# Sthiber/COSC_4397_Pathtracing_Raytracing_Project

Hardware: AMD Instinct MI355X
Metric: Msamples/s, cornell.txt 1920x1080 depth 8 (+PSNR vs 5000spp ref) (higher is better)
Workload: dtype f32

## Files before the change

cosc_4397_pathtracing_raytracing_project_amd/capi.py:

```python
from __future__ import annotations

import ctypes as C
import math
import os
from typing import Optional, Sequence, Tuple

import numpy as np

_PKG = os.path.dirname(os.path.abspath(__file__))
LIB_PATH = os.environ.get("PT_AMD_LIB") or os.path.join(_PKG, "libpt_amd.so")
PT_MAX_DEPTH = 64
ARITH = {"exact": 0, "fma": 1, "fast": 2}
ARITH_NAMES = {v: k for k, v in ARITH.items()}
FEATURE_PLANES = 3
NOISE_PLANES = 2
NOISE_PIXELS_PER_PARTIAL = 1024
CONVERGENCE_WAVES = 16
CONVERGENCE_CAPACITY = 65536
FLT_MAX = float(np.finfo(np.float32).max)


class PtGeom(C.Structure):
    _fields_ = [("type", C.c_int32), ("materialid", C.c_int32), ("transform", C.c_float * 16),
                ("inverseTransform", C.c_float * 16), ("invTranspose", C.c_float * 16)]


class PtMaterial(C.Structure):
    _fields_ = [("color", C.c_float * 3), ("specular_exponent", C.c_float), ("specular_color", C.c_float * 3),
                ("hasReflective", C.c_float), ("hasRefractive", C.c_float), ("indexOfRefraction", C.c_float),
                ("emittance", C.c_float)]


class PtCamera(C.Structure):
    _fields_ = [("resolution", C.c_int32 * 2), ("position", C.c_float * 3), ("lookAt", C.c_float * 3),
                ("view", C.c_float * 3), ("up", C.c_float * 3), ("right", C.c_float * 3), ("fov", C.c_float * 2),
                ("pixelLength", C.c_float * 2)]


class PtBVHNode(C.Structure):
    _fields_ = [("bmin", C.c_float * 3), ("bmax", C.c_float * 3), ("left", C.c_int32), ("right", C.c_int32),
                ("geomIndex", C.c_int32)]


class PtGridInfo(C.Structure):
    _fields_ = [("res", C.c_int32 * 3), ("origin", C.c_float * 3), ("cell_size", C.c_float * 3), ("pad", C.c_float),
                ("num_cells", C.c_int32), ("num_records", C.c_int32), ("num_leaves", C.c_int32)]


class PtGridRecord(C.Structure):
    _fields_ = [("bmin", C.c_float * 3), ("bmax", C.c_float * 3), ("leaf", C.c_int32), ("neighbours", C.c_int32)]


class PtCameraGridResult(C.Structure):
    _fields_ = [("res", C.c_int32 * 3), ("origin", C.c_float * 3), ("cell_size", C.c_float * 3), ("inv_cell_size", C.c_float * 3), ("pad", C.c_float),
                ("guard", C.c_uint32), ("num_cells", C.c_int64), ("refs", C.c_uint64), ("longest", C.c_uint32), ("status", C.c_int32)]


class PtSceneDesc(C.Structure):
    _fields_ = [("geoms", C.POINTER(PtGeom)), ("num_geoms", C.c_int32), ("materials", C.POINTER(PtMaterial)),
                ("num_materials", C.c_int32), ("camera", PtCamera), ("trace_depth", C.c_int32)]


class PtOptions(C.Structure):
    _fields_ = [("device", C.c_int32), ("pixel_begin", C.c_int32), ("pixel_count", C.c_int32),
                ("iters_per_batch", C.c_int32), ("num_queues", C.c_int32), ("blocks_per_cu", C.c_int32),
                ("time_kernels", C.c_int32), ("legacy_traversal", C.c_int32), ("debug_flags", C.c_int32), ("unfused_primary", C.c_int32), ("unfused_bounces", C.c_int32), ("stripe_pixels", C.c_int32), ("stripe_stride", C.c_int32),
                ("arith", C.c_int32), ("aa_jitter", C.c_int32), ("convergence", C.c_int32),
                ("lds_table_kb", C.c_int32), ("primary_pieces", C.c_int32), ("paths_pieces", C.c_int32), ("paths_min_piece", C.c_int32)]


class PtStats(C.Structure):
    _fields_ = [("samples", C.c_int64), ("live_rays", C.c_int64 * PT_MAX_DEPTH), ("intersect_launches", C.c_int64),
                ("intersect_ms", C.c_double), ("render_ms", C.c_double), ("num_cus", C.c_int32),
                ("grid_blocks", C.c_int32), ("num_queues", C.c_int32), ("iters_per_batch", C.c_int32),
                ("device_bytes", C.c_int64), ("primary_fused", C.c_int32), ("bounces_fused", C.c_int32),
                ("arith", C.c_int32), ("grid_cells", C.c_int32), ("tight_leaves", C.c_int32), ("paths_waves", C.c_int32), ("record_form", C.c_int32),
                ("gather_form", C.c_int32), ("primary_launches", C.c_int64), ("inline_gathers", C.c_int64)]


class PtDenoiseOptions(C.Structure):
    _fields_ = [("levels", C.c_int32), ("sigma_color", C.c_float), ("sigma_normal", C.c_float), ("sigma_position", C.c_float),
                ("keep_albedo", C.c_int32)]


class PtHistoryOptions(C.Structure):
    _fields_ = [("cap", C.c_float), ("min_normal_dot", C.c_float), ("plane_tol", C.c_float), ("keep_view_dependent", C.c_int32)]


class PtHistoryRoundOptions(C.Structure):
    _fields_ = [("min_history", C.c_float), ("max_fraction", C.c_float)]


class PtHistoryProbeOptions(C.Structure):
    _fields_ = [("radius", C.c_int32), ("gain", C.c_float)]


class PtHistoryFeedbackOptions(C.Structure):
    _fields_ = [("level", C.c_int32), ("variance", C.c_int32)]


class PtSetupTimes(C.Structure):
    _fields_ = [("tables_ms", C.c_double), ("upload_ms", C.c_double), ("buffers_ms", C.c_double), ("probe_ms", C.c_double),
                ("set_camera_ms", C.c_double), ("set_camera_calls", C.c_int32)]


class PtSetCameraTimes(C.Structure):
    _fields_ = [("tables_ms", C.c_double), ("rearm_ms", C.c_double), ("total_ms", C.c_double), ("path", C.c_int32), ("fallback", C.c_int32)]


class PtSetGeomsTimes(C.Structure):
    _fields_ = [("build_ms", C.c_double), ("upload_ms", C.c_double), ("rearm_ms", C.c_double), ("total_ms", C.c_double)]


PT_SET_CAMERA_DEVICE_TABLES = 1
PT_DEVICE_TABLES_LIST, PT_DEVICE_TABLES_CELLS = 1, 2
PT_CAMERA_GRID_NONE = 3
TABLE_NODE = np.dtype([("bmin", np.float32, 3), ("bmax", np.float32, 3), ("skip", np.int32), ("geom", np.int32)])
TABLE_NAMES = ("nodes", "nodes_b", "top", "top_b", "grid_start", "grid_items", "grid_items_b", "cull_margin", "geoms")


class PtError(RuntimeError):
    pass


_lib: Optional[C.CDLL] = None
_fp = C.POINTER(C.c_float)
_ip = C.POINTER(C.c_int32)


def lib() -> C.CDLL:
    global _lib
    if _lib is not None:
        return _lib
    if not os.path.exists(LIB_PATH):
        raise PtError(f"{LIB_PATH} not found: run `python -c 'import __graft_entry__ as g; g.build()'` "
                      "(hipcc --offload-arch=gfx950).  There is no CPU fallback.")
    L = C.CDLL(LIB_PATH)
    L.pt_last_error.restype = C.c_char_p
    L.pt_scene_load.argtypes = [C.c_char_p, C.c_int, C.c_int, C.POINTER(C.c_void_p)]
    L.pt_scene_free.argtypes = [C.c_void_p]
    L.pt_scene_free.restype = None
    L.pt_scene_desc.argtypes = [C.c_void_p, C.POINTER(PtSceneDesc)]
    L.pt_scene_iterations.argtypes = [C.c_void_p]
    L.pt_scene_image_name.argtypes = [C.c_void_p]
    L.pt_scene_image_name.restype = C.c_char_p
    L.pt_build_bvh.argtypes = [C.POINTER(PtGeom), C.c_int, C.POINTER(PtBVHNode), C.c_int]
    L.pt_build_grid.argtypes = [C.POINTER(PtGeom), C.c_int, C.c_int, C.POINTER(PtGridInfo), C.POINTER(C.c_uint32), C.POINTER(PtGridRecord)]
    if hasattr(L, "pt_selfcheck_ieee"):
        L.pt_selfcheck_ieee.argtypes = [C.c_int, C.c_int, C.c_uint64, C.c_uint64, C.c_uint32, C.POINTER(C.c_uint64)]
    if hasattr(L, "pt_selfcheck_fast_math"):
        L.pt_selfcheck_fast_math.argtypes = [C.c_int, C.c_int, C.c_uint64, C.c_uint64, C.POINTER(C.c_double)]
    if hasattr(L, "pt_traversal_boxes"):
        L.pt_traversal_boxes.argtypes = [C.POINTER(PtGeom), C.c_int, _fp, _fp]
    if hasattr(L, "pt_center_half_box"):
        L.pt_center_half_box.argtypes = [_fp, _fp, C.c_int, C.c_float, _fp, _fp]
        L.pt_center_half_box.restype = None
    L.pt_build_transform.argtypes = [_fp, _fp, _fp, _fp]
    L.pt_init.argtypes = [C.POINTER(PtSceneDesc), C.POINTER(PtOptions)]
    L.pt_render.argtypes = [C.c_int, C.c_int]
    L.pt_readback.argtypes = [_fp]
    L.pt_readback_device.argtypes = [C.c_void_p]
    L.pt_preview_rgba8.argtypes = [C.c_int, C.POINTER(C.c_uint8)]
    L.pt_preview_rgba8_device.argtypes = [C.c_int, C.c_void_p]
    L.pt_get_stats.argtypes = [C.POINTER(PtStats)]
    L.pt_stage_generate.argtypes = [C.c_int, C.c_int, _fp, _fp]
    L.pt_stage_intersect.argtypes = [C.c_int, _fp, _fp, _fp, _fp, _ip, _fp]
    if hasattr(L, "pt_stage_intersect_grid"):
        L.pt_stage_intersect_grid.argtypes = [C.c_int, _fp, _fp, C.c_int, _fp, _fp, _ip, _fp]
        L.pt_stage_grid_info.argtypes = [C.POINTER(PtGridInfo), C.POINTER(C.c_int32)]
    L.pt_stage_shade.argtypes = [C.c_int, C.c_int, _ip, _ip, _fp, _fp, _ip, _fp, _fp, _fp, _fp, _ip]
    _u8p = C.POINTER(C.c_uint8)
    L.pt_save_u8.argtypes = [C.c_float, _u8p]
    L.pt_stage_save_u8.argtypes = [C.c_int, C.c_int, C.c_float, _fp, _u8p]
    L.pt_ctx_create.argtypes = [C.POINTER(PtSceneDesc), C.POINTER(PtOptions), C.POINTER(C.c_void_p)]
    L.pt_ctx_destroy.argtypes = [C.c_void_p]
    L.pt_ctx_render.argtypes = [C.c_void_p, C.c_int, C.c_int]
    L.pt_ctx_sync.argtypes = [C.c_void_p]
    L.pt_ctx_readback.argtypes = [C.c_void_p, _fp]
    L.pt_ctx_readback_device.argtypes = [C.c_void_p, C.c_void_p]
    L.pt_ctx_save_u8.argtypes = [C.c_void_p, C.c_float, _u8p]
    L.pt_ctx_get_stats.argtypes = [C.c_void_p, C.POINTER(PtStats)]
    L.pt_ctx_reset_stats.argtypes = [C.c_void_p]
    L.pt_ctx_clear.argtypes = [C.c_void_p]
    L.pt_ctx_pixel_count.argtypes = [C.c_void_p]
    L.pt_group_create.argtypes = [C.POINTER(PtSceneDesc), C.POINTER(PtOptions), _ip, C.c_int, C.POINTER(C.c_void_p)]
    if hasattr(L, "pt_group_create_ex"):
        L.pt_group_create_ex.argtypes = [C.POINTER(PtSceneDesc), C.POINTER(PtOptions), _ip, C.c_int, C.c_int, C.POINTER(C.c_void_p)]
        L.pt_group_transport.argtypes = [C.c_void_p]
    L.pt_group_destroy.argtypes = [C.c_void_p]
    L.pt_group_size.argtypes = [C.c_void_p]
    L.pt_group_context.argtypes = [C.c_void_p, C.c_int]
    L.pt_group_context.restype = C.c_void_p
    L.pt_group_render.argtypes = [C.c_void_p, C.c_int, C.c_int]
    L.pt_group_sync.argtypes = [C.c_void_p]
    L.pt_group_gather.argtypes = [C.c_void_p, _fp]
    L.pt_group_gather_u8.argtypes = [C.c_void_p, C.c_float, _u8p]
    L.pt_group_preview_rgba8.argtypes = [C.c_void_p, C.c_int, _u8p]
    L.pt_write_png_rgb8.argtypes = [C.c_char_p, _u8p, C.c_int, C.c_int]
    L.pt_output_basename.argtypes = [C.c_char_p, C.c_int, C.c_char_p, C.c_int]
    L.pt_save_png.argtypes = [C.c_char_p, _fp, C.c_int, C.c_int, C.c_float]
    L.pt_save_hdr.argtypes = [C.c_char_p, _fp, C.c_int, C.c_int, C.c_float]
    L.pt_save_pfm.argtypes = [C.c_char_p, _fp, C.c_int, C.c_int, C.c_float]
    L.pt_load_pfm.argtypes = [C.c_char_p, _fp, C.c_int, _ip, _ip, C.c_float]
    _dp = C.POINTER(C.c_double)
    L.pt_psnr_from_sse.argtypes = [C.c_double, C.c_int64]
    L.pt_psnr_from_sse.restype = C.c_float
    L.pt_set_reference.argtypes = [_fp]
    L.pt_get_convergence.argtypes = [C.c_int, C.c_int, _dp]
    L.pt_iterations_to_clean.argtypes = [C.c_float, _ip]
    L.pt_ctx_set_reference.argtypes = [C.c_void_p, _fp]
    L.pt_ctx_get_convergence.argtypes = [C.c_void_p, C.c_int, C.c_int, _dp]
    L.pt_ctx_iterations_to_clean.argtypes = [C.c_void_p, C.c_float, _ip]
    L.pt_group_set_reference.argtypes = [C.c_void_p, _fp]
    L.pt_group_get_convergence.argtypes = [C.c_void_p, C.c_int, C.c_int, _dp]
    L.pt_group_iterations_to_clean.argtypes = [C.c_void_p, C.c_float, _ip]
    if hasattr(L, "pt_render_features"):
        L.pt_render_features.argtypes = [C.c_int, C.c_int]
        L.pt_readback_features.argtypes = [_fp]
        L.pt_ctx_render_features.argtypes = [C.c_void_p, C.c_int, C.c_int]
        L.pt_ctx_readback_features.argtypes = [C.c_void_p, _fp]
        L.pt_ctx_device_features.argtypes = [C.c_void_p]
        L.pt_ctx_device_features.restype = C.c_void_p
        L.pt_group_render_features.argtypes = [C.c_void_p, C.c_int, C.c_int]
        L.pt_group_gather_features.argtypes = [C.c_void_p, _fp]
    if hasattr(L, "pt_denoise"):
        _dno = C.POINTER(PtDenoiseOptions)
        L.pt_denoise.argtypes = [C.c_float, _dno, _fp]
        L.pt_ctx_denoise.argtypes = [C.c_void_p, C.c_float, _dno, _fp]
        L.pt_ctx_denoise_device.argtypes = [C.c_void_p, C.c_float, _dno, C.POINTER(C.c_void_p)]
        L.pt_group_denoise.argtypes = [C.c_void_p, C.c_float, _dno, _fp]
# ... 1898 lines not shown
```

cosc_4397_pathtracing_raytracing_project_amd/csrc/pt_api.cpp:

```cpp
#include <chrono>
#include <cmath>
#include <cstdarg>
#include <cstdio>
#include <cstring>
#include <string>

#include "pt_adaptive.h"
#include "pt_camera_tables_device.h"
#include "pt_context.h"
#include "pt_lds.h"
#include "pt_scene.h"
#include "pt_sched.h"

namespace {

std::string g_err;
constexpr int kDebugFlags = 16 | 32 | 64 | 256 | 512 | 2048 | ptk::kFormSwitches;
static_assert(sizeof(PtOptions) == 80, "capi.PtOptions mirrors this layout");
static_assert(PT_CONVERGENCE_WAVES == ptk::kConvWaves, "pt_amd.h documents the size of the convergence metric's partial sums");
}
int pt_fail(const char* fmt, ...) {
  char buf[1024];
  va_list ap;
  va_start(ap, fmt);
  vsnprintf(buf, sizeof(buf), fmt, ap);
  va_end(ap);
  g_err = buf;
  return -1;
}

namespace ptc {
static PtContext* g_default = nullptr;
PtContext* default_context() { return g_default; }

int get_events(Ctx& g, EventPair* ev) {
  if (!g.free_events.empty()) {
    *ev = g.free_events.back();
    g.free_events.pop_back();
    return 0;
  }
  HIP_OK(hipEventCreate(&ev->a));
  HIP_OK(hipEventCreate(&ev->b));
  return 0;
}
static int resolve_events(Ctx& g) {
  auto drain = [&](std::vector<EventPair>& pending, double& total_ms) -> int {
    for (auto& e : pending) {
      float ms = 0;
      HIP_OK(hipEventElapsedTime(&ms, e.a, e.b));
      total_ms += ms;
      g.free_events.push_back(e);
    }
    pending.clear();
    return 0;
  };
  g.isect_launches += (int64_t)g.pending_isect.size();
  return drain(g.pending_isect, g.isect_ms) || drain(g.pending_render, g.render_ms) ? -1 : 0;
}

ptk::SceneTables tables(const Ctx& g) {
  ptk::SceneTables t = g.scene;
  if (g.debug_flags & 16) t.cull_margin = INFINITY;
  if (g.debug_flags & 32) t.top_xor = 0;
  t.lds_table_bytes = g.lds_table_bytes;
  t.max_batch_iters = g.K;
  t.trace_depth = g.depth;
  t.scan_nodes_lds = -1;
  t.use_grid = !g.grids.empty() && g.grid_enabled && !(g.debug_flags & 512) ? 1 : 0;
  if (t.use_grid) {
    const Ctx::DeviceGrid& gr = g.grids[g.grid_pick];
    t.lds_table_bytes = -1;
    t.grid_start = gr.d_start + gr.guard;
    t.grid_items = gr.d_items;
    t.grid_items_b = gr.d_items_b;
    for (int a = 0; a < 3; ++a)
      t.grid_res[a] = gr.shape.res[a], t.grid_min[a] = gr.shape.gmin[a], t.grid_cs[a] = gr.shape.cs[a], t.grid_inv_cs[a] = gr.shape.inv_cs[a];
    t.grid_pad = gr.shape.pad;
  }
  return t;
}

static size_t pathbuf_words(int64_t stride) { return (size_t)(2 * stride + (stride * ptd::kPathPlane2Bytes + 15) / 16); }
static int alloc_pathbuf(Ctx& g, ptd::PathBuf* b, int64_t stride) {
  b->stride = stride;
  return dalloc(g, &b->r, pathbuf_words(stride));
}
static int alloc_hitbuf(Ctx& g, ptd::HitBuf* h, int64_t stride) {
  h->stride = stride;
  return dalloc(g, &h->t, stride) || dalloc(g, &h->n, 3 * stride) || dalloc(g, &h->mat, stride) || dalloc(g, &h->p, 3 * stride) ? -1 : 0;
}

static ptd::Queues queues_for(const Ctx& g, int grid) {
  ptd::Queues q = g.qs;
  q.W = grid * ptk::kWavesPerBlock;
  return q;
}

static int primary_share_of(const Ctx& g) { return (g.debug_flags & ptk::kTraceEveryIteration) ? 1 : g.primary_share ? g.primary_share : ptk::kShareMax; }

ptk::BatchInfo tile_batch(const Ctx& g, int iter_first, int K) {
  ptk::BatchInfo b{};
  b.iter_first = iter_first;
  b.K = K;
  b.N = g.N;
  b.pixel_begin = g.pixel_begin;
  b.trace_depth = g.depth;
  b.aa_jitter = g.aa_jitter ? 1 : 0;
  b.stripe = g.stripe;
  b.gap = g.stripe ? g.stripe_stride - g.stripe : 0;
  b.inv_stripe = g.stripe ? 1.0f / (float)g.stripe : 0.0f;
  return b;
}
static ptk::BatchInfo form_batch(const Ctx& g, int iter_first, int K) {
  ptk::BatchInfo b = tile_batch(g, iter_first, K);
  b.slot_shift = g.slot_shift, b.flat = g.fuse_bounces ? 0 : 1, b.primary_share = primary_share_of(g);
  return b;
}

static void gather_waiting(Ctx& g) {
  if (!g.waiting.live) return;
  ptd::RetireBuf ret = g.ret;
  if (g.waiting.plane) ret.rec = g.rec_plane1;
  g.k->collect_stream_planes(g.stream, g.waiting.b, g.qs, ret, g.ret.rec, g.d_image);
  g.waiting.live = false;
}

int run_batch(Ctx& g, int iter_first, int kb, int after) {
  ptk::BatchInfo b = form_batch(g, iter_first, kb);
  b.paths_pieces = g.paths_pieces, b.list = g.list;
  if (b.list) b.stripe = 1, b.gap = 0, b.inv_stripe = 1.0f;
  const ptk::SceneTables sc = tables(g);
  const ptk::BatchForm form = ptk::batch_form(ptk::form_inputs(b, g.debug_flags, ptk::search_form(sc), sc.num_mats, g.ret.seg_cap));
  b.retire_once = form.retire_once, b.split_records = g.record_form = form.records, b.fixed_slots = form.fixed_slots;
  b.primary_pieces = form.shares ? ptk::auto_shared_pieces(kb, g.qs.nq, g.ret.wq0) : ptk::auto_primary_pieces(kb, g.qs.nq, g.ret.wq0);
  if (g.primary_pieces) b.primary_pieces = g.primary_pieces;
  if (form.records == ptk::kFirstBounce) b.primary_pieces = 1;
  const ptk::KernelApi& k = *g.k;
  auto cnt_row = [&](int d) { return g.d_cnt + ptk::cnt_index(g.qs, d, 0); };
  const ptd::Queues pq = queues_for(g, g.grid_primary);
  Ctx::PrimaryKey key;
  std::memset(&key, 0, sizeof(key));
  key.sc = sc, key.cam = g.dcam, key.b = b, key.b.iter_first = key.b.K = 0, key.qs = pq, key.out = g.buf[1], key.ret = g.ret;
  key.kernels = &k, key.grid = g.grid_primary, key.debug_flags = g.debug_flags;
  const bool same_key = form.primary_once && g.primary_valid && std::memcmp(&key, &g.primary_key, sizeof(key)) == 0;
  g.primary_valid = false;
  ptk::ConvInfo cv{g.d_ref, g.d_partial, -1, kb};
  if (g.conv_live) {
    if (g.conv_have_ref) cv.first_k = 0;
    else if (g.conv >= iter_first && g.conv < iter_first + kb) cv.capture_k = g.conv - iter_first, cv.first_k = cv.capture_k + 1, g.conv_have_ref = true;
    g.conv_last = std::max(g.conv_last, iter_first + kb - 1);
  }
  const bool all_depths = g.grid_paths > 0;
  const ptk::GatherPlan plan = ptk::gather_plan({form, cv.capture_k >= 0 || cv.first_k < kb, g.waiting.live, g.waiting.plane, same_key,
                                                 g.rec_plane1 != nullptr && !g.conv, after, g.debug_flags, all_depths});
  ptd::RetireBuf ret = g.ret;
  if (plan.plane) ret.rec = g.rec_plane1;
  if (!plan.gathers_waiting) gather_waiting(g);
  if (!g.fuse_primary) k.generate(g.stream, g.grid_gen, g.dcam, b, queues_for(g, g.grid_gen), g.buf[0], cnt_row(0));
  else if (!same_key) {
    k.primary(g.stream, g.grid_primary, sc, g.dcam, b, pq, cnt_row(0), cnt_row(1), g.buf[1], g.ret);
    g.primary_launches += 1;
    std::memcpy(&g.primary_key, &key, sizeof(key));
  }
  const int d0 = g.fuse_primary ? 1 : 0;
  int src = d0;
  EventPair ev{};
  auto timed_from = [&]() -> int {
    if (!g.time_kernels) return 0;
    if (get_events(g, &ev)) return -1;
    HIP_OK(hipEventRecord(ev.a, g.stream));
    return 0;
  };
  auto timed_to = [&]() -> int {
    if (!g.time_kernels) return 0;
    HIP_OK(hipEventRecord(ev.b, g.stream));
    g.pending_isect.push_back(ev);
    return 0;
  };
  if (all_depths) {
    if (timed_from()) return -1;
    if (plan.gathers_waiting) {
      const ptk::PrevGather prev{g.waiting.plane ? g.rec_plane1 : g.ret.rec, g.ret.rec, g.d_image, g.waiting.b.K, 0};
      k.paths_gather(g.stream, g.grid_paths, sc, b, queues_for(g, g.grid_paths), g.d_cnt, g.buf[1], ret, prev);
      g.waiting.live = false;
      g.inline_gathers += 1;
    } else k.paths(g.stream, g.grid_paths, sc, b, queues_for(g, g.grid_paths), g.d_cnt, g.buf[1], ret);
    if (timed_to()) return -1;
  }
  for (int d = d0; d < g.depth && !all_depths; ++d) {
    const int32_t* cin = cnt_row(d);
    int32_t* cout = cnt_row(d + 1);
    if (timed_from()) return -1;
    k.intersect(g.stream, g.grid_isect, sc, queues_for(g, g.grid_isect), cin, g.buf[src], g.hits, g.legacy, d == 0);
    if (timed_to()) return -1;
    k.shade(g.stream, g.grid_shade, sc, b, d, queues_for(g, g.grid_shade), cin, cout, g.buf[src], g.hits, g.buf[src ^ 1], g.ret);
    src ^= 1;
  }
  g.gather_form = plan.reported;
  if (plan.closing == ptk::kCloseStream) k.collect_stream(g.stream, b, g.qs, g.ret, g.d_image, g.d_cnt, g.depth, g.d_stats);
  else k.count_stats(g.stream, g.qs, g.d_cnt, g.depth, g.d_stats);
  if (plan.closing == ptk::kCloseStatsStreamPlanes) k.collect_stream_planes(g.stream, b, g.qs, ret, g.ret.rec, g.d_image);
  if (plan.closing == ptk::kCloseStatsConv) k.collect_conv(g.stream, b, g.qs, g.ret, g.d_image, cv, g.d_sse);
  if (plan.closing == ptk::kCloseStatsTile) k.collect(g.stream, b, g.qs, g.ret, g.d_image);
  if (plan.defers) g.waiting.live = true, g.waiting.b = b, g.waiting.plane = plan.plane;
  HIP_OK(hipGetLastError());
  g.primary_valid = form.primary_once;
  g.samples += (int64_t)kb * g.N;
  if (g.pending_isect.size() > 16384) {
    HIP_OK(hipStreamSynchronize(g.stream));
    if (resolve_events(g)) return -1;
  }
  return 0;
}

void plan_launch(Ctx& g) {
  if (!g.borrowed) g.lds_table_bytes = g.k->lds_table_limit(tables(g), g.lds_table_forced);
  const ptk::SceneTables t = tables(g);
  g.grid_gen = g.num_cus * std::min(g.cap_bpc, g.k->resident_blocks_per_cu(ptk::kGenerate, t));
  g.grid_isect = g.num_cus * std::min(g.cap_bpc, g.k->resident_blocks_per_cu(g.legacy ? ptk::kIntersectLegacy : ptk::kIntersect, t));
  g.grid_shade = g.num_cus * std::min(g.cap_bpc, g.k->resident_blocks_per_cu(ptk::kShade, t));
  g.grid_primary = g.num_cus * std::min(g.cap_bpc, g.k->resident_blocks_per_cu(ptk::primary_shares(form_batch(g, 0, g.K)) ? ptk::kPrimaryShared : ptk::kPrimary, t));
  g.ret.wq0 = ptk::wave_slot(0, g.qs.Q, g.grid_primary * ptk::kWavesPerBlock).wq;
  g.grid_paths = (g.fuse_bounces && g.depth > 1) ? g.num_cus * std::min(g.cap_bpc, g.k->resident_blocks_per_cu(ptk::kPaths, t)) : 0;
  g.qs.paths_W = g.grid_paths * ptk::kWavesPerBlock;
  g.primary_valid = false;
}

static void free_grid(Ctx& g, const Ctx::DeviceGrid& d) {
  for (void* p : {(void*)d.d_start, (void*)d.d_items, d.d_items_b != d.d_items ? (void*)d.d_items_b : nullptr}) {
    if (!p) continue;
    (void)hipFree(p);
    g.allocs.erase(std::remove(g.allocs.begin(), g.allocs.end(), p), g.allocs.end());
  }
  g.device_bytes -= (int64_t)d.bytes;
}
static int choose_traversal(Ctx& g) {
  auto drop_unused_grids = [&](size_t keep) {
    for (size_t i = 0; i < g.grids.size(); ++i)
      if (i != keep) free_grid(g, g.grids[i]);
    g.grids = {g.grids[keep]};
    g.grid_pick = 0;
  };
  if (g.grids.empty()) return 0;
  if (!g.fuse_bounces || (g.debug_flags & (256 | 512))) {
    drop_unused_grids(0);
    return 0;
  }
// ... 104 lines not shown
  auto pieces = [](int v, int automatic) { return v ? std::clamp(v, 1, 0x7fff) : automatic; };
  g.lds_table_forced = opt.lds_table_kb ? std::clamp(opt.lds_table_kb, 0, ptk::kLdsTableBytes / 1024) * 1024 : -1;
  g.primary_pieces = pieces(opt.primary_pieces < 0 ? opt.primary_pieces : opt.primary_pieces & 0xffff, 0);
  g.primary_share = opt.primary_pieces < 0 ? 0 : std::min(opt.primary_pieces >> 16 & 0x7f, ptk::kShareMax);
  g.paths_pieces = ptk::pack_paths_pieces(pieces(opt.paths_pieces, 2), pieces(opt.paths_min_piece, 64));
  g.fuse_primary = !g.legacy && !opt.unfused_primary;
  g.fuse_bounces = g.fuse_primary && !opt.unfused_bounces;
  g.cap_bpc = opt.blocks_per_cu > 0 ? std::min(opt.blocks_per_cu, 8) : 8;
}

int batch_iters_for(int iters_per_batch, int N, int* slot_shift) {
  int K = iters_per_batch;
  if (K <= 0) {
    const int64_t target = 48ll << 20;
    K = (int)std::max<int64_t>(1, std::min<int64_t>(256, (target + N - 1) / N));
  }
  int shift = 1;
  while ((1ll << shift) < N) ++shift;
  if (shift > 30) return pt_fail("pt_init: tiles of more than 2^30 pixels are not supported");
  while (K > 1 && K > (1 << (31 - shift))) --K;
  if (slot_shift) *slot_shift = shift;
  return K;
}

int plan_batches(Ctx& g, const PtOptions& opt) {
  const int W = g.cam.resolution[0], H = g.cam.resolution[1];
  g.opt_iters_per_batch = opt.iters_per_batch, g.opt_num_queues = opt.num_queues;
  g.pixel_begin = opt.pixel_begin;
  g.N = opt.pixel_count > 0 ? opt.pixel_count : W * H - opt.pixel_begin;
  g.stripe = opt.stripe_pixels;
  g.stripe_stride = opt.stripe_stride;
  if (g.stripe < 0 || (g.stripe > 0 && g.stripe_stride < g.stripe)) return pt_fail("pt_init: bad stripe %d / stride %d", g.stripe, g.stripe_stride);
  {
    int64_t last = (int64_t)g.pixel_begin + g.N - 1;
    if (g.stripe > 0) last = (int64_t)g.pixel_begin + (g.N - 1) + (int64_t)((g.N - 1) / g.stripe) * (g.stripe_stride - g.stripe);
    if (g.pixel_begin < 0 || g.N <= 0 || last >= (int64_t)W * H)
      return pt_fail("pt_init: tile [%d, +%d, stripe %d/%d) outside %dx%d", opt.pixel_begin, opt.pixel_count, g.stripe, g.stripe_stride, W, H);
    if (g.stripe > 0 && g.N / g.stripe >= 32768) return pt_fail("pt_init: more than 32767 stripes");
    if (H >= 32768) return pt_fail("pt_init: image height %d not supported (>= 32768)", H);
  }
  const int K = batch_iters_for(opt.iters_per_batch, g.N, &g.slot_shift);
  if (K < 0) return -1;

  int Q = opt.num_queues > 0 ? opt.num_queues : 256;
  const int cu_waves = g.num_cus * ptk::kWavesPerBlock;
  if (Q > cu_waves) Q = cu_waves;
  while (cu_waves % Q) --Q;
  if (opt.num_queues <= 0)
    while (ptk::chunks_per_queue(g.N, Q) > 128 && 2 * Q <= cu_waves && cu_waves % (2 * Q) == 0) Q *= 2;
  const ptk::QueuePlan plan = ptk::queue_plan(g.N, Q, K);
  const int grid = g.num_cus * 8;
  g.K = K;
  g.grid = grid;
  g.qs.Q = Q;
  g.qs.W = grid * ptk::kWavesPerBlock;
  g.qs.cnt_stride = 16;
  g.qs.nq = plan.nq;
  g.qs.inv_nq = 1.0f / (float)plan.nq;
  g.qs.cap = plan.cap;
  g.stride = (int64_t)Q * g.qs.cap;
  g.ret.seg_cap = plan.seg_cap;
  g.ret.kmax = K;
  return 0;
}

template <typename T>
static const T* upload(Ctx& g, const std::vector<T>& v) {
  T* p = nullptr;
  if (dalloc(g, &p, v.size())) return nullptr;
  const hipError_t e = hipMemcpy(p, v.data(), v.size() * sizeof(T), hipMemcpyHostToDevice);
  return e == hipSuccess ? p : (pt_fail("hipMemcpy(%zu bytes) failed: %s", v.size() * sizeof(T), hipGetErrorString(e)), nullptr);
}
static int upload_grid(Ctx& g, const pt::Grid& gr) {
  Ctx::DeviceGrid d{gr.shape, gr.guard, nullptr, nullptr, nullptr, 0, gr.start};
  const int64_t before = g.device_bytes;
  if (!(d.d_start = upload(g, gr.start)) || !(d.d_items = upload(g, gr.items))) return -1;
  if (!(d.d_items_b = gr.items_b.empty() ? d.d_items : upload(g, gr.items_b))) return -1;
  d.bytes = (size_t)(g.device_bytes - before);
  d.items = gr.items.size();
  g.grids.push_back(d);
  return 0;
}
static int upload_tables(Ctx& g, const pt::HostTables& t) {
  ptk::SceneTables& s = g.scene;
  s.num_nodes = (int)t.nodes.size(), s.num_geoms = (int)t.geoms.size(), s.num_mats = (int)t.mats.size(), s.num_top = (int)t.top.size();
  std::memcpy(s.root_min, t.root_min, 12);
  std::memcpy(s.root_max, t.root_max, 12);
  s.cull_margin = t.cull_margin;
  s.top_xor = t.top_xor;
  s.has_triangles = t.has_triangles ? 1 : 0;
  g.tight_leaves = t.tight_leaves;
  if (!(s.nodes = upload(g, t.nodes)) || !(s.geoms = upload(g, t.geoms)) || !(s.mats = upload(g, t.mats)) || !(s.top = upload(g, t.top))) return -1;
  s.nodes_b = s.nodes, s.top_b = s.top;
  if (!t.nodes_b.empty() && (!(s.nodes_b = upload(g, t.nodes_b)) || !(s.top_b = upload(g, t.top_b)))) return -1;
  for (const pt::Grid& gr : t.grids)
    if (upload_grid(g, gr)) return -1;
  return 0;
}

static __global__ void k_poison_records(ptd::Word4* rec, unsigned long long per_queue, unsigned long long total, int Q) {
  const float nan = __builtin_nanf("");
  for (unsigned long long i = (unsigned long long)blockIdx.x * blockDim.x + threadIdx.x; i < total; i += (unsigned long long)gridDim.x * blockDim.x)
    rec[i] = ptd::Word4{nan, nan, nan, __int_as_float(ptk::chunk_pixel((int)(i / per_queue), 0, Q))};
}

static int poison_records(Ctx& g) {
  const size_t regions = (size_t)g.qs.Q * g.ret.kmax, per_queue = (size_t)g.ret.kmax * g.ret.seg_cap;
  for (ptd::Word4* plane : {g.ret.rec, g.rec_plane1})
    if (plane)
      hipLaunchKernelGGL(k_poison_records, dim3((unsigned)std::min<size_t>((regions * g.ret.seg_cap + 255) / 256, 65536)), dim3(256), 0, g.stream, plane,
                         (unsigned long long)per_queue, (unsigned long long)(regions * g.ret.seg_cap), g.qs.Q);
  HIP_OK(hipGetLastError());
  return 0;
}
static size_t sub_words_max(const Ctx& g) { return ptk::sub_stride(g.num_cus * 8 * ptk::kWavesPerBlock, g.qs.Q); }

static int rearm_batch_buffers(Ctx& g) {
  g.primary_valid = false;
  for (const ptd::PathBuf& pb : g.buf) HIP_OK(hipMemsetAsync(pb.r, 0xff, pathbuf_words(pb.stride) * sizeof(ptd::Word4), g.stream));
  const size_t regions = (size_t)g.qs.Q * g.ret.kmax;
  HIP_OK(hipMemsetAsync(g.ret.cnt, 0, regions * sizeof(*g.ret.cnt), g.stream));
  HIP_OK(hipMemsetAsync(g.ret.sub, 0, regions * sub_words_max(g) * sizeof(*g.ret.sub), g.stream));
  if (g.qs.deal) HIP_OK(hipMemsetAsync(g.qs.deal, 0, (size_t)ptk::deal_map(g.qs).words() * sizeof(int32_t), g.stream));
  return poison_records(g);
}

int alloc_batch_buffers(Ctx& g) {
  const int Q = g.qs.Q;
  if (alloc_pathbuf(g, &g.buf[0], g.stride) || alloc_pathbuf(g, &g.buf[1], g.stride)) return -1;
  for (const ptd::PathBuf& pb : g.buf) HIP_OK(hipMemset(pb.r, 0xff, pathbuf_words(pb.stride) * sizeof(ptd::Word4)));
  if (!g.fuse_bounces && alloc_hitbuf(g, &g.hits, g.stride)) return -1;
  {
    const size_t regions = (size_t)Q * g.ret.kmax;
    const size_t wq_max = sub_words_max(g);
    if (dalloc(g, &g.ret.rec, regions * g.ret.seg_cap)) return -1;
    g.rec_plane1 = nullptr;
    if (g.fuse_primary && g.fuse_bounces && g.depth > 1 && !g.aa_jitter && !g.borrowed && !(g.debug_flags & ptk::kNoSecondPlane)) {
      void* p = nullptr;
      const size_t bytes = regions * g.ret.seg_cap * sizeof(ptd::Word4);
      if (hipMalloc(&p, bytes) == hipSuccess) {
        g.allocs.push_back(p);
        g.device_bytes += (int64_t)bytes;
        g.rec_plane1 = static_cast<ptd::Word4*>(p);
      } else (void)hipGetLastError();
    }
    if (ensure(g, g.ret.cnt, regions * sizeof(*g.ret.cnt), Zero::blocking) || ensure(g, g.ret.sub, regions * wq_max * sizeof(*g.ret.sub), Zero::blocking)) return -1;
    if (poison_records(g)) return -1;
  }
  const size_t image_bytes = 3 * (size_t)g.N * sizeof(float);
  const size_t cnt_words = ptk::cnt_index(g.qs, g.depth + 1, 0);
  if (ensure(g, g.d_image, image_bytes, Zero::blocking) || ensure(g, g.d_cnt, cnt_words * sizeof(int32_t), Zero::blocking) ||
      ensure(g, g.d_stats, PT_MAX_DEPTH * sizeof(*g.d_stats), Zero::blocking))
    return -1;
  if (!(g.debug_flags & 64) && ensure(g, g.qs.deal, (size_t)ptk::deal_map(g.qs).words() * sizeof(int32_t), Zero::blocking)) return -1;
  if (g.conv) {
    const size_t partials = (size_t)g.K * Q * ptk::kConvWaves;
    if (ensure(g, g.d_ref, image_bytes, Zero::blocking) || ensure(g, g.d_partial, partials * sizeof(double), Zero::blocking)) return -1;
    if (dalloc(g, &g.d_sse, (size_t)PT_CONVERGENCE_CAPACITY)) return -1;
    HIP_OK(hipMemset(g.d_sse, 0xff, (size_t)PT_CONVERGENCE_CAPACITY * sizeof(double)));
  }
  HIP_OK(hipDeviceSynchronize());
  return 0;
}

static int setup(Ctx& g, const PtSceneDesc* sc, const PtOptions& opt) {
  if (open_device(g, opt)) return -1;
  take_scene_and_options(g, sc, opt);
  if (plan_batches(g, opt)) return -1;
  if ((size_t)sc->num_materials * sizeof(ptd::Mat) > 60 * 1024) return pt_fail("pt_init: %zu materials exceed the LDS table", (size_t)sc->num_materials);
  using clock = std::chrono::steady_clock;
  auto ms_since = [](clock::time_point t0) { return std::chrono::duration<double, std::milli>(clock::now() - t0).count(); };
  clock::time_point t0 = clock::now();
  const pt::HostTables host = pt::build_scene_tables(*sc, g.debug_flags, g.k->boxes_center_half != 0, pt::GridRequest{}, &g.camera_base);
  g.setup_times.tables_ms = ms_since(t0), t0 = clock::now();
  if (upload_tables(g, host)) return -1;
  g.setup_times.upload_ms = ms_since(t0), t0 = clock::now();
  plan_launch(g);
  if (alloc_batch_buffers(g)) return -1;
  g.setup_times.buffers_ms = ms_since(t0), t0 = clock::now();
  if (choose_traversal(g)) return -1;
  g.setup_times.probe_ms = ms_since(t0);
  g.grid_request.kind = pt::GridRequest::kNone;
  if (tables(g).use_grid) {
    g.grid_request.kind = pt::GridRequest::kFixed;
    std::memcpy(g.grid_request.res, g.grids[g.grid_pick].shape.res, sizeof(g.grid_request.res));
  }
  g.time_kernels = opt.time_kernels != 0;
  g.conv_live = g.conv != 0;
  return 0;
}

int need(const PtContext* c, const char* who) { return c ? 0 : pt_fail("%s: pt_init has not been called", who); }

int admit(const PtContext& g, const char* who, unsigned req) {
  if ((req & kNotFailed) && g.failed) return pt_fail("%s: an earlier batch of this context failed (%s); free it and create a new one", who, g_err.c_str());
  if ((req & kUniform) && g.adaptive)
    return pt_fail("%s: the renderer is in the adaptive state (pt_adaptive_round): one sample count no longer describes the image; read it with pt_resolve, or "
                   "return to the uniform state with pt_clear", who);
  if ((req & kNoExtras) && g.hist_extra)
    return pt_fail("%s: the history round left extra samples in some pixels (pt_history_round): one sample count no longer describes the image; read it with "
                   "pt_history_resolve, or return to the uniform state with pt_clear", who);
  const int W = g.cam.resolution[0];
  if ((req & kWholeRows) && (g.stripe || g.pixel_begin % W || g.N % W))
    return pt_fail("%s: the tile must consist of whole contiguous image rows (begin %d, count %d, stripe %d, width %d)", who, g.pixel_begin, g.N, g.stripe, W);
  if ((req & kFoldedAll) && g.rendered != g.noise_iters)
    return pt_fail("%s: %lld iteration(s) rendered since the last fold; fold first (pt_noise_fold)", who, (long long)(g.rendered - g.noise_iters));
  if (req & kOnDevice) HIP_OK(hipSetDevice(g.device));
  return 0;
}

}
using namespace ptc;

extern "C" {

const char* pt_last_error(void) { return g_err.c_str(); }

int pt_selfcheck_ieee(int arith, int kind, uint64_t first, uint64_t count, uint32_t seed, uint64_t* mismatches) {
  const ptk::KernelApi* k = ptk::api_for(arith);
  if (!k || kind < 0 || kind > 4 || !mismatches) return pt_fail("pt_selfcheck_ieee: bad argument");
  unsigned long long* d = nullptr;
  HIP_OK(hipMalloc(&d, sizeof(*d)));
  hipError_t e = hipMemset(d, 0, sizeof(*d));
  if (e == hipSuccess) {
    k->ieee_check(nullptr, kind, first, count, seed, d);
    e = hipGetLastError();
  }
  unsigned long long h = 0;
  if (e == hipSuccess) e = hipMemcpy(&h, d, sizeof(h), hipMemcpyDeviceToHost);
  (void)hipFree(d);
  if (e != hipSuccess) return pt_fail("pt_selfcheck_ieee: %s", hipGetErrorString(e));
  *mismatches = h;
  return 0;
}

int pt_selfcheck_fast_math(int arith, int kind, uint64_t first, uint64_t count, double* max_err) {
  const ptk::KernelApi* k = ptk::api_for(arith);
  if (!k || kind < 0 || kind > 8 || !max_err) return pt_fail("pt_selfcheck_fast_math: bad argument");
  unsigned long long* d = nullptr;
  HIP_OK(hipMalloc(&d, sizeof(*d)));
  hipError_t e = hipMemset(d, 0, sizeof(*d));
  if (e == hipSuccess) {
    k->fast_math_check(nullptr, kind, first, count, d);
    e = hipGetLastError();
  }
  unsigned long long h = 0;
  if (e == hipSuccess) e = hipMemcpy(&h, d, sizeof(h), hipMemcpyDeviceToHost);
  (void)hipFree(d);
  if (e != hipSuccess) return pt_fail("pt_selfcheck_fast_math: %s", hipGetErrorString(e));
  std::memcpy(max_err, &h, sizeof(h));
  return 0;
}

struct PtScene {
  pt::Scene scene;
  explicit PtScene(const std::string& f) : scene(f) {}
};

int pt_scene_load(const char* path, int res_w, int res_h, PtScene** out) {
  if (!path || !out) return pt_fail("pt_scene_load: null argument");
  try {
    PtScene* s = new PtScene(path);
    if (res_w > 0 && res_h > 0) s->scene.overrideResolution(res_w, res_h);
    s->scene.applyInitialCameraState();
    *out = s;
    return 0;
  } catch (const std::exception& e) {
    return pt_fail("pt_scene_load: %s", e.what());
  }
}
void pt_scene_free(PtScene* s) { delete s; }
int pt_scene_desc(const PtScene* s, PtSceneDesc* out) {
  if (!s || !out) return pt_fail("pt_scene_desc: null argument");
  *out = s->scene.desc();
  return 0;
}
int pt_scene_orbit(PtScene* s, float dphi, float dtheta, float dzoom) {
  if (!s) return pt_fail("pt_scene_orbit: null scene");
  s->scene.orbit(dphi, dtheta, dzoom);
  return 0;
}
int pt_scene_camera(const PtScene* s, PtCamera* out) {
  if (!s || !out) return pt_fail("pt_scene_camera: null argument");
  *out = s->scene.state.camera;
  return 0;
}
int pt_scene_orbit_state(const PtScene* s, float* phi, float* theta, float* zoom) {
  if (!s) return pt_fail("pt_scene_orbit_state: null scene");
  if (phi) *phi = s->scene.phi;
  if (theta) *theta = s->scene.theta;
  if (zoom) *zoom = s->scene.zoom;
  return 0;
}
static int scene_geom(const PtScene* s, int geom, const void* trs, const char* who) {
  if (!s || !trs) return pt_fail("%s: null argument", who);
  if (geom < 0 || (size_t)geom >= s->scene.geoms.size()) return pt_fail("%s: geom %d is outside the scene's %zu geoms", who, geom, s->scene.geoms.size());
  if (s->scene.geom_trs[(size_t)geom].mesh) return pt_fail("%s: geom %d is a triangle of a mesh object: its vertices are world-space, it has no TRS of its own", who, geom);
  return 0;
}
int pt_scene_geom_trs(const PtScene* s, int geom, float trs[9]) {
  if (scene_geom(s, geom, trs, "pt_scene_geom_trs")) return -1;
  std::memcpy(trs, s->scene.geom_trs[(size_t)geom].trs, 9 * sizeof(float));
  return 0;
}
int pt_scene_set_geom_trs(PtScene* s, int geom, const float trs[9]) {
  if (scene_geom(s, geom, trs, "pt_scene_set_geom_trs")) return -1;
  for (int k = 0; k < 9; ++k)
// ... 59 lines not shown
  if (!sc) return pt_fail("pt_init: null scene");
  if (sc->num_geoms <= 0 || !sc->geoms) return pt_fail("pt_init: scene has no geometry");
  if (sc->num_materials <= 0 || !sc->materials) return pt_fail("pt_init: scene has no materials");
  if (sc->trace_depth <= 0 || sc->trace_depth > PT_MAX_DEPTH) return pt_fail("pt_init: trace_depth %d out of range", sc->trace_depth);
  const int W = sc->camera.resolution[0], H = sc->camera.resolution[1];
  if (W <= 0 || H <= 0 || (int64_t)W * H > (1ll << 30)) return pt_fail("pt_init: bad resolution %dx%d", W, H);
  for (int i = 0; i < sc->num_geoms; ++i) {
    if (sc->geoms[i].materialid < 0 || sc->geoms[i].materialid >= sc->num_materials)
      return pt_fail("pt_init: geom %d references material %d of %d", i, sc->geoms[i].materialid, sc->num_materials);
    if (sc->geoms[i].type < PT_GEOM_SPHERE || sc->geoms[i].type > PT_GEOM_TRIANGLE)
      return pt_fail("pt_init: geom %d has unknown type %d", i, sc->geoms[i].type);
  }
  PtOptions opt{};
  if (opt_in) opt = *opt_in;
  PtContext* c = new PtContext();
  if (setup(*c, sc, opt)) {
    destroy(c);
    return -1;
  }
  *out = c;
  return 0;
}

int pt_ctx_destroy(PtContext* c) {
  if (c == g_default) g_default = nullptr;
  destroy(c);
  return 0;
}

int pt_ctx_render(PtContext* c, int iter_first, int iter_count) {
  if (need(c, "pt_render")) return -1;
  if (iter_count <= 0) return 0;
  Ctx& g = *c;
  if (admit(g, "pt_render", kNotFailed | kUniform)) return -1;
  if (g.conv_live) {
    if (iter_first < 1 || (int64_t)iter_first + iter_count - 1 > PT_CONVERGENCE_CAPACITY)
      return pt_fail("pt_render: iterations %d .. %lld outside 1 .. %d (PT_CONVERGENCE_CAPACITY) with the convergence metric on", iter_first,
                  (long long)iter_first + iter_count - 1, PT_CONVERGENCE_CAPACITY);
    if (g.conv < 0 && !g.conv_have_ref) return pt_fail("pt_render: PtOptions.convergence is -1 but no reference frame has been supplied (pt_set_reference)");
  }
  HIP_OK(hipSetDevice(g.device));
  EventPair ev{};
  if (get_events(g, &ev)) return -1;
  HIP_OK(hipEventRecord(ev.a, g.stream));
  const int end = iter_first + iter_count;
  for (int it = iter_first; it < end; it += g.K)
    if (run_batch(g, it, std::min(g.K, end - it), it + g.K < end ? (end - it - 1) / g.K : 0)) {
      g.failed = true;
      g.free_events.push_back(ev);
      return -1;
    }
  HIP_OK(hipEventRecord(ev.b, g.stream));
  g.pending_render.push_back(ev);
  g.rendered += iter_count;
  g.fb_pending = false;
  return 0;
}

int pt_ctx_sync(PtContext* c) {
  if (need(c, "pt_sync")) return -1;
  HIP_OK(hipSetDevice(c->device));
  HIP_OK(hipStreamSynchronize(c->stream));
  return resolve_events(*c);
}

int pt_ctx_readback(PtContext* c, float* out) {
  if (need(c, "pt_readback")) return -1;
  return copy_out(c, "pt_readback", out, 3, [&](const float** d) { return *d = c->d_image, 0; });
}

int pt_ctx_readback_device(PtContext* c, void* out) {
  if (need(c, "pt_readback_device")) return -1;
  return copy_out(c, "pt_readback_device", static_cast<float*>(out), 3, [&](const float** d) { return *d = c->d_image, 0; }, hipMemcpyDeviceToDevice);
}

const float* pt_ctx_device_image(PtContext* c) { return c ? c->d_image : nullptr; }
void* pt_ctx_stream(PtContext* c) { return c ? (void*)c->stream : nullptr; }
int pt_ctx_pixel_count(const PtContext* c) { return c ? c->N : 0; }
int pt_ctx_device(const PtContext* c) { return c ? c->device : -1; }

int pt_ctx_save_u8_device(PtContext* c, float samples, const uint8_t** rgb8_dev) {
  if (need(c, "pt_save_u8")) return -1;
  Ctx& g = *c;
  const int W = g.cam.resolution[0];
  if (!(samples > 0.0f)) return pt_fail("pt_save_u8: samples must be positive");
  if (admit(g, "pt_save_u8", kUniform | kNoExtras)) return -1;
  if (g.pixel_begin % W || g.N % W || (g.stripe && g.stripe != W))
    return pt_fail("pt_save_u8: the tile must consist of whole image rows (begin %d, count %d, stripe %d, width %d)", g.pixel_begin, g.N, g.stripe, W);
  HIP_OK(hipSetDevice(g.device));
  if (ensure(g, g.d_rgb8, 3 * (size_t)g.N)) return -1;
  g.k->save_u8(g.stream, g.N, W, samples, g.d_image, g.d_rgb8);
  HIP_OK(hipGetLastError());
  if (rgb8_dev) *rgb8_dev = g.d_rgb8;
  return 0;
}
int pt_ctx_save_u8(PtContext* c, float samples, uint8_t* rgb8_host) {
  return copy_out(c, "pt_save_u8", rgb8_host, 3, [&](const uint8_t** d) { return pt_ctx_save_u8_device(c, samples, d); });
}

int pt_ctx_preview_rgba8_device(PtContext* c, int iterations, void* rgba_dev) {
  if (need(c, "pt_preview_rgba8_device")) return -1;
  if (!rgba_dev || iterations <= 0) return pt_fail("pt_preview_rgba8_device: bad argument");
  if (admit(*c, "pt_preview_rgba8_device", kUniform | kNoExtras | kOnDevice)) return -1;
  c->k->preview(c->stream, c->N, iterations, c->d_image, reinterpret_cast<uchar4*>(rgba_dev));
  HIP_OK(hipStreamSynchronize(c->stream));
  return 0;
}

int pt_ctx_preview_rgba8(PtContext* c, int iterations, uint8_t* rgba_host) {
  if (need(c, "pt_preview_rgba8")) return -1;
  if (!rgba_host || iterations <= 0) return pt_fail("pt_preview_rgba8: bad argument");
  if (admit(*c, "pt_preview_rgba8", kUniform | kNoExtras | kOnDevice)) return -1;
  uchar4* d = nullptr;
  HIP_OK(hipMalloc((void**)&d, (size_t)c->N * 4));
  c->k->preview(c->stream, c->N, iterations, c->d_image, d);
  hipError_t e = hipMemcpyAsync(rgba_host, d, (size_t)c->N * 4, hipMemcpyDeviceToHost, c->stream);
  if (e == hipSuccess) e = hipStreamSynchronize(c->stream);
  (void)hipFree(d);
  if (e != hipSuccess) return pt_fail("pt_preview_rgba8: %s", hipGetErrorString(e));
  return 0;
}

int pt_ctx_get_stats(PtContext* c, PtStats* out) {
  if (need(c, "pt_get_stats")) return -1;
  if (!out) return pt_fail("pt_get_stats: null");
  if (pt_ctx_sync(c)) return -1;
  Ctx& g = *c;
  std::memset(out, 0, sizeof(*out));
  unsigned long long st[PT_MAX_DEPTH];
  HIP_OK(hipMemcpy(st, g.d_stats, sizeof(st), hipMemcpyDeviceToHost));
  for (int d = 0; d < PT_MAX_DEPTH; ++d) out->live_rays[d] = (int64_t)st[d];
  out->samples = g.samples;
  out->intersect_launches = g.isect_launches;
  out->intersect_ms = g.isect_ms;
  out->render_ms = g.render_ms;
  out->num_cus = g.num_cus;
  out->grid_blocks = g.grid_paths > 0 ? g.grid_paths : g.grid_isect;
  out->num_queues = g.qs.Q;
  out->iters_per_batch = g.K;
  out->device_bytes = g.device_bytes;
  out->primary_fused = g.fuse_primary ? 1 : 0;
  out->bounces_fused = g.fuse_bounces ? 1 : 0;
  out->arith = g.arith;
  if (tables(g).use_grid && g.fuse_bounces) {
    const int* res = g.grids[g.grid_pick].shape.res;
    out->grid_cells = res[0] * res[1] * res[2];
  }
  out->tight_leaves = g.tight_leaves;
  out->record_form = g.record_form;
  out->gather_form = g.gather_form;
  out->inline_gathers = g.inline_gathers;
  out->primary_launches = g.primary_launches;
  out->paths_waves = 0;
  if (g.qs.deal && g.grid_paths > 0) {
    const ptk::DealMap dm = ptk::deal_map(g.qs);
    std::vector<int32_t> first((size_t)dm.made_for() + 1);
    HIP_OK(hipMemcpy(first.data(), g.qs.deal + dm.first(0), first.size() * sizeof(int32_t), hipMemcpyDeviceToHost));
    if (first[dm.made_for()] == g.qs.paths_W) {
      int lo = first[1] - first[0], hi = lo;
      for (int q = 1; q < g.qs.Q; ++q) lo = std::min(lo, first[q + 1] - first[q]), hi = std::max(hi, first[q + 1] - first[q]);
      out->paths_waves = std::min(lo, 0xffff) << 16 | std::min(hi, 0xffff);
    }
  }
  return 0;
}

int pt_ctx_reset_stats(PtContext* c) {
  if (need(c, "pt_reset_stats")) return -1;
  if (pt_ctx_sync(c)) return -1;
  Ctx& g = *c;
  HIP_OK(hipMemsetAsync(g.d_stats, 0, PT_MAX_DEPTH * sizeof(unsigned long long), g.stream));
  HIP_OK(hipStreamSynchronize(g.stream));
  g.samples = 0;
  g.isect_ms = g.render_ms = 0;
  g.isect_launches = 0;
  return 0;
}

int pt_ctx_clear(PtContext* c) {
  if (need(c, "pt_clear")) return -1;
  if (pt_ctx_sync(c)) return -1;
  HIP_OK(hipMemsetAsync(c->d_image, 0, 3 * (size_t)c->N * sizeof(float), c->stream));
  if (c->d_feat) HIP_OK(hipMemsetAsync(c->d_feat, 0, (size_t)PT_FEATURE_PLANES * c->N * sizeof(float4), c->stream));
  if (c->d_noise) HIP_OK(hipMemsetAsync(c->d_noise, 0, pt_noise_state_bytes((size_t)c->N), c->stream));
  c->noise_groups = 0;
  c->noise_iters = c->rendered = 0;
  if (c->d_acnt) HIP_OK(hipMemsetAsync(c->d_acnt, 0, (size_t)c->N * sizeof(ptad::Cnt), c->stream));
  c->adaptive = false;
  c->adaptive_rounds = 0;
  c->adaptive_last = 0;
  c->hist_current = c->feat_fresh = false;
  c->hist_var_current = 0;
  c->fb_current = c->fb_pending = false;
  if (c->d_hist_extra) HIP_OK(hipMemsetAsync(c->d_hist_extra, 0, (size_t)c->N * sizeof(float), c->stream));
  c->hist_extra = false;
  c->hist_noise = c->hist_ne = false;
  c->probe_checked = c->probe_applied = false;
  if (c->conv) {
    HIP_OK(hipMemsetAsync(c->d_sse, 0xff, (size_t)PT_CONVERGENCE_CAPACITY * sizeof(double), c->stream));
    c->conv_last = 0;
    if (c->conv > 0) c->conv_have_ref = false;
  }
  return pt_ctx_reset_stats(c);
}

}
int pt_ctx_camera_refusal(const PtContext* c, const PtCamera* cam, const char* who) {
  if (need(c, who) || admit(*c, who, kNotFailed)) return -1;
  if (!cam) return pt_fail("%s: null camera", who);
  if (cam->resolution[0] != c->cam.resolution[0] || cam->resolution[1] != c->cam.resolution[1])
    return pt_fail("%s: resolution %dx%d differs from the renderer's %dx%d; a new resolution needs pt_init", who, cam->resolution[0], cam->resolution[1],
                   c->cam.resolution[0], c->cam.resolution[1]);
  const struct {
    const char* name;
    const float* v;
    int n;
  } fields[] = {{"position", cam->position, 3}, {"view", cam->view, 3}, {"up", cam->up, 3}, {"right", cam->right, 3}, {"fov", cam->fov, 2}, {"pixelLength", cam->pixelLength, 2}};
  for (const auto& f : fields)
    for (int i = 0; i < f.n; ++i)
      if (!std::isfinite(f.v[i])) return pt_fail("%s: camera %s[%d] is not finite", who, f.name, i);
  return 0;
}
int pt_ctx_camera_refusal_ex(const PtContext* c, const PtCamera* cam, uint32_t flags, const char* who) {
  if (need(c, who) || admit(*c, who, kNotFailed)) return -1;
  if (!cam) return pt_fail("%s: null camera", who);
  if (flags & ~(uint32_t)PT_SET_CAMERA_DEVICE_TABLES) return pt_fail("%s: undefined flag bit(s) 0x%x (defined: PT_SET_CAMERA_DEVICE_TABLES = 0x%x)", who, flags & ~(uint32_t)PT_SET_CAMERA_DEVICE_TABLES, PT_SET_CAMERA_DEVICE_TABLES);
  return pt_ctx_camera_refusal(c, cam, who);
}
int pt_ctx_geoms_refusal(const PtContext* c, const PtGeom* geoms, int num_geoms, const char* who) {
  if (need(c, who) || admit(*c, who, kNotFailed)) return -1;
  if (!geoms) return pt_fail("%s: null geoms", who);
  const std::vector<PtGeom>& have = c->camera_base.geoms;
  if (num_geoms != (int)have.size())
    return pt_fail("%s: %d geoms, but the renderer was created with %d; adding or removing objects needs pt_init", who, num_geoms, (int)have.size());
  for (int i = 0; i < num_geoms; ++i)
    if (geoms[i].type != have[(size_t)i].type || geoms[i].materialid != have[(size_t)i].materialid)
      return pt_fail("%s: geom %d has type %d and material %d, the renderer's has type %d and material %d; only the transforms may change", who, i, geoms[i].type,
                     geoms[i].materialid, have[(size_t)i].type, have[(size_t)i].materialid);
  for (int i = 0; i < num_geoms; ++i)
    for (const float* m : {geoms[i].transform, geoms[i].inverseTransform, geoms[i].invTranspose})
      for (int k = 0; k < 16; ++k)
        if (!std::isfinite(m[k])) return pt_fail("%s: geom %d has a matrix element that is not finite", who, i);
  return 0;
}
namespace {
template <typename T>
void release(Ctx& g, const T* dev, size_t count) {
  if (!dev) return;
  void* p = const_cast<T*>(dev);
  (void)hipFree(p);
  g.allocs.erase(std::remove(g.allocs.begin(), g.allocs.end(), p), g.allocs.end());
  g.device_bytes -= (int64_t)std::max<size_t>(count * sizeof(T), 16);
}
template <typename T>
int reupload(const T* dev, const std::vector<T>& v) {
  HIP_OK(hipMemcpy(const_cast<T*>(dev), v.data(), v.size() * sizeof(T), hipMemcpyHostToDevice));
  return 0;
}
int move_grid(Ctx& g, const pt::Grid* gr) {
  if (!g.grids.empty()) {
    Ctx::DeviceGrid& d = g.grids[g.grid_pick];
    if (gr && gr->start.size() == d.start.size() && gr->items.size() == d.items && gr->items_b.empty() == (d.d_items_b == d.d_items)) {
      if (reupload(d.d_start, gr->start) || reupload(d.d_items, gr->items)) return -1;
      if (!gr->items_b.empty() && reupload(d.d_items_b, gr->items_b)) return -1;
      d.shape = gr->shape, d.guard = gr->guard, d.start = gr->start, d.start_stale = false;
      return 0;
    }
    free_grid(g, d);
    g.grids.clear();
    g.grid_pick = 0;
  }
  return gr ? upload_grid(g, *gr) : 0;
}
int move_tables(Ctx& g) {
  pt::HostTables t;
  std::memcpy(t.root_min, g.scene.root_min, 12);
  std::memcpy(t.root_max, g.scene.root_max, 12);
  const bool center_half = g.k->boxes_center_half != 0;
  pt::camera_tables(t, g.camera_base, g.cam.position, g.debug_flags, center_half, g.grid_request);
  ptk::SceneTables& s = g.scene;
  if (reupload(s.nodes, t.nodes) || reupload(s.top, t.top)) return -1;
  if (center_half && (reupload(s.nodes_b, t.nodes_b) || reupload(s.top_b, t.top_b))) return -1;
  s.cull_margin = t.cull_margin;
  g.tight_leaves = t.tight_leaves;
  return move_grid(g, t.grids.empty() ? nullptr : &t.grids[0]);
}


int ensure_device_base(Ctx& g) {
  Ctx::DeviceBase& b = g.device_base;
  if (b.ready) return 0;
  const pt::CameraBase& cb = g.camera_base;
  std::vector<ptct::DeviceGeom> geoms(cb.geoms.size());
  for (size_t i = 0; i < geoms.size(); ++i) {
    geoms[i] = ptct::DeviceGeom{};
    std::memcpy(geoms[i].inv, cb.geoms[i].inverseTransform, sizeof(geoms[i].inv));
    geoms[i].type = cb.geoms[i].type;
  }
  if (!(b.nodes = upload(g, cb.nodes)) || !(b.top = upload(g, cb.top)) || !(b.geoms = upload(g, geoms))) return -1;
  if (b.rec) return b.ready = true, 0;
  if (dalloc(g, &b.rec, 1)) return -1;
  if (g.grid_request.kind == pt::GridRequest::kFixed) {
    int64_t ncell = 1, leaves = 0;
    for (int a = 0; a < 3; ++a) ncell *= std::min(512, std::max(1, g.grid_request.res[a]));
    for (const ptd::Node& n : cb.nodes) leaves += n.geom >= 0 ? 1 : 0;
    if (ncell <= ptct::kDeviceMaxCells) {
// ... 400 lines not shown
```

cosc_4397_pathtracing_raytracing_project_amd/csrc/pt_device.h:

```cpp
#pragma once
#include <stdint.h>

namespace ptd {

struct Node {
  float bmin[3];
  float bmax[3];
  int32_t skip;
  int32_t geom;
};
static_assert(sizeof(Node) == 32, "Node must be 32 B");

constexpr int kMaxTop = 32;
struct TopEntry {
  float bmin[3];
  float bmax[3];
  int32_t idx;
  int32_t link;
};
static_assert(sizeof(TopEntry) == 32, "TopEntry must be 32 B");

struct Geom {
  float inv[12];
  float xf[12];
  float invT[12];
  int32_t type;
  int32_t material;
  int32_t pad[2];
  float box_normal[7][4];
};
static_assert(sizeof(Geom) == 272, "Geom must be 272 B");

struct Mat {
  float color[3];
  float spec[3];
  float reflective;
  float refractive;
  float emittance;
  float pad[3];
};
static_assert(sizeof(Mat) == 48, "Mat must be 48 B");

struct Camera {
  int32_t res_x, res_y;
  float pos[3], view[3], up[3], right[3];
  float pl_x, pl_y;
};

struct alignas(16) Word4 {
  float x, y, z, w;
};
constexpr int kPathPlane2Bytes = 8;
struct PathBuf {
  Word4* r;
  int64_t stride;
};
struct HitBuf {
  float* t;
  float* n;
  int32_t* mat;
  float* p;
  int64_t stride;
};

struct RetireBuf {
  Word4* rec;
  unsigned long long* sub;
  unsigned long long* cnt;
  int32_t seg_cap;
  int32_t kmax;
  int32_t wq0;
  int32_t pad;
};

struct Queues {
  int32_t Q;
  int32_t cap;
  int32_t W;
  int32_t cnt_stride;
  int32_t nq;
  float inv_nq;
  int32_t* deal;
  int32_t paths_W;
  int32_t pad;
};

}
```

cosc_4397_pathtracing_raytracing_project_amd/csrc/pt_kernels.hip:

```cpp
#include "pt_kernels.h"

#include <float.h>

#include <type_traits>

#include "pt_lds.h"
#include "pt_sched.h"
#include "pt_portable_math.h"

#ifndef PT_ARITH
#define PT_ARITH 0
#endif
#if PT_ARITH == 0
#define PT_NS arith_exact
#define PT_API_FN api_exact
#elif PT_ARITH == 1
#define PT_NS arith_fma
#define PT_API_FN api_fma
#elif PT_ARITH == 2
#define PT_NS arith_fast
#define PT_API_FN api_fast
#else
#error "PT_ARITH must be 0, 1 or 2"
#endif
// ... 1186 lines not shown
      "global_load_lds_dwordx4 %[o16], %[b1]\n\t"
      "s_add_u32 m0, m0, 0x400\n\t"
      "s_nop 0\n\t"
      "global_load_lds_dword %[o8], %[b2]\n\t"
      "s_add_u32 m0, m0, 0xfc\n\t"
      "s_nop 0\n\t"
      "global_load_lds_dword %[o8], %[b2] offset:4\n\t"
      "s_mov_b32 m0, %[keep]"
      : [keep] "=&s"(keep)
      : [base] "s"(lds_base), [b0] "s"(b0), [b1] "s"(b1), [b2] "s"(b2), [o16] "v"(off16), [o8] "v"(off8)
      : "memory", "scc");
}
PT_DEV void fetch_split_to_lds(const void* b0, const void* b1, int i, int i0, uint32_t lds_base) {
  uint32_t keep;
  const uint32_t off = (uint32_t)i << 4, off0 = (uint32_t)i0 << 4;
  asm volatile(
      "s_mov_b32 %[keep], m0\n\t"
      "s_mov_b32 m0, %[base]\n\t"
      "s_nop 0\n\t"
      "global_load_lds_dwordx4 %[o], %[b0]\n\t"
      "s_add_u32 m0, m0, 0x400\n\t"
      "s_nop 0\n\t"
      "global_load_lds_dwordx4 %[o0], %[b1]\n\t"
      "s_mov_b32 m0, %[keep]"
      : [keep] "=&s"(keep)
      : [base] "s"(lds_base), [b0] "s"(b0), [b1] "s"(b1), [o] "v"(off), [o0] "v"(off0)
      : "memory", "scc");
}
PT_DEV void read_record_slot(uint32_t s16, uint32_t s4, v4f& w0, v4f& w1, float& cz, int& nslot, int& nrs) {
  asm volatile(
      "s_waitcnt vmcnt(0)\n\t"
      "ds_read_b128 %0, %5\n\t"
      "ds_read_b128 %1, %5 offset:1024\n\t"
      "ds_read_b32 %2, %6\n\t"
      "ds_read_b32 %3, %6 offset:256\n\t"
      "ds_read_b32 %4, %6 offset:512\n\t"
      "s_waitcnt lgkmcnt(0)"
      : "=&v"(w0), "=&v"(w1), "=&v"(cz), "=&v"(nslot), "=&v"(nrs)
      : "v"(s16), "v"(s4)
      : "memory");
}
struct Lanes {
  unsigned long long* best;
  float* rec;
  uint16_t* ent;
  int head, count;
  int appended, processed;
};
PT_DEV Lanes lanes_init(char* base) {
  Lanes c;
  c.best = reinterpret_cast<unsigned long long*>(base + LanesMap::best);
  c.rec = reinterpret_cast<float*>(base + LanesMap::rec);
  c.ent = reinterpret_cast<uint16_t*>(base + LanesMap::ent);
  c.head = c.count = c.appended = c.processed = 0;
  return c;
}
PT_DEV void paths_chunk(Lanes& c, int n, int lane, f3 o, f3 d, const uint32_t* tword, const ptd::Geom* __restrict__ geoms) {
  const bool valid = lane < n;
  const uint32_t entry = c.ent[(c.head + lane) & (kRing - 1)];
  const int src = (int)(entry & 63u);
  const uint32_t tw = tword[valid ? entry >> 6 : 0u];
  const uint32_t leaf = tw & 255u;
  const f3 ro = mk(bperm(src, o.x), bperm(src, o.y), bperm(src, o.z));
  const f3 rd = mk(bperm(src, d.x), bperm(src, d.y), bperm(src, d.z));
  const ptd::Geom* G = geoms + (valid ? (int)(tw >> 8) : 0);
  f3 pt = mk(0.f, 0.f, 0.f), nrm = mk(0.f, 0.f, 0.f);
  const float t = geom_test<-1, false>(G, ro, rd, pt, nrm, mk(0.f, 0.f, 0.f));
  const uint32_t tb = __float_as_uint(t);
  if (valid && t > 0.f && tb < 0x7f7fffffu) {
    const unsigned long long key = ((unsigned long long)tb << 32) | leaf;
    unsigned long long* slot = &c.best[src];
    atomicMin(slot, key);
    if (*slot == key) {
      float* r = c.rec + src;
      r[0 * 64] = nrm.x, r[1 * 64] = nrm.y, r[2 * 64] = nrm.z;
      r[3 * 64] = pt.x, r[4 * 64] = pt.y, r[5 * 64] = pt.z;
    }
  }
  c.head = (c.head + n) & (kRing - 1);
  c.count -= n;
  c.processed += n;
}
typedef __attribute__((address_space(4))) const v4f cfloat4;
template <typename TOP>
PT_DEV void paths_search(Lanes& c, TOP* top, const uint32_t* tword, int ntop, const ptd::Geom* __restrict__ geoms, f3 o, f3 d,
                         bool fresh, int lane, int& mark) {
  const RayInv ri = ray_inv(d, o);
  if (fresh) {
    c.best[lane] = kNoHit;
    mark = c.processed;
  }
  uint32_t mask = 0;
  for (int e0 = 0; e0 < ntop; e0 += 8) {
#pragma unroll
    for (int u = 0; u < 8; ++u) {
      const int e = e0 + u;
      if (e < ntop) {
        const auto A = top[2 * e], B = top[2 * e + 1];
        mask = push_bit(mask, slab(o, ri, A.x, A.y, A.z, A.w, B.x, B.y));
      }
    }
  }
  mask = fresh ? mask : 0u;
  while (true) {
    const unsigned long long m = ballot(mask != 0u);
    if (!m) break;
    const int rank = rank_in(m);
    if (mask != 0u) {
      const int te = ntop - 1 - __builtin_ctz(mask);
      mask &= mask - 1u;
      c.ent[(c.head + c.count + rank) & (kRing - 1)] = (uint16_t)((te << 6) | lane);
      if (mask == 0u) mark = c.appended + rank + 1;
    }
    const int cnt = __popcll(m);
    c.count += cnt;
    c.appended += cnt;
    if (c.count >= 64) paths_chunk(c, 64, lane, o, d, tword, geoms);
  }
}
constexpr int kPathsScanWaves = 5, kPathsGridWaves = 5;
constexpr int kVisitLap = 32, kVisitsPerRefill = 31;
static_assert(kVisitLap + kVisitsPerRefill + 1 <= kVisitRing, "the visit ring laps a path in flight");
static_assert((kVisitRing & (kVisitRing - 1)) == 0, "visit numbers wrap with a mask");
constexpr int kInlineGroup = 8;
template <int GROUP>
PT_DEV void stream_gather_slot(int N, int K, const QueueShare& sh, const ptd::RetireBuf& ret, const ptd::Word4* plane, const ptd::Word4* front,
                               float* __restrict__ image, int q, int s);
template <typename... PREV>
struct PathsPrev {};
template <typename P>
struct PathsPrev<P> {
  P p;
};
template <typename... PREV>
struct PathsArgs {
  SceneTables sc;
  BatchInfo b;
  ptd::Queues qs;
  int32_t* cnt;
  ptd::PathBuf in;
  ptd::RetireBuf ret;
  PathsPrev<PREV...> prev;
};
template <typename A>
PT_DEV const A& cold_args() {
  auto p = __builtin_amdgcn_kernarg_segment_ptr();
  asm volatile("" : "+s"(p));
  return *(const A*)p;
}
PT_DEV int cold(int v) {
  asm volatile("" : "+s"(v));
  return v;
}
template <Search MODE, int SPLIT = 0, typename... PREV>
__global__ __launch_bounds__(kBlock, MODE == 0 ? kPathsWaves : MODE == 1 ? kPathsScanWaves : kPathsGridWaves) void k_paths(SceneTables sc, BatchInfo b, ptd::Queues qs, int32_t* __restrict__ cnt ,
                                                               ptd::PathBuf in, ptd::RetireBuf ret, PREV... prev) {
  extern __shared__ float4 lds_raw[];
  char* lds = reinterpret_cast<char*>(lds_raw);
  const PathsLds L = paths_lds<MODE, kFast>(sc);
  stage16(lds + L.top, sc.top_b, MODE == 2 ? 0 : top_bytes(sc));
  stage16(lds + L.mats, sc.mats, mat_bytes(sc));
  const float4* top = reinterpret_cast<const float4*>(lds + L.top);
  const ptd::Mat* mats = reinterpret_cast<const ptd::Mat*>(lds + L.mats);
  const ptd::Node* nodes = sc.nodes_b;
  const ptd::Geom* geoms = sc.geoms;
  if (MODE == 0) {
    stage16(lds + L.geoms, sc.geoms, geom_bytes(sc));
    geoms = reinterpret_cast<const ptd::Geom*>(lds + L.geoms);
  }
  const char* lnodes = nullptr;
  if (MODE == 1 && sc.scan_nodes_lds > 0) {
    stage16(lds + L.nodes, sc.nodes_b, node_bytes(sc));
    lnodes = lds + L.nodes;
  }
  using WM = PathsWaveMap<MODE, kFast>;
  constexpr bool FIXED = SPLIT == kFixedSlots, FIRST = SPLIT == kFirstBounce || FIXED;
  constexpr bool GATHER = sizeof...(PREV) > 0;
  static_assert(!GATHER || FIXED, "only a batch with fixed record slots gathers its predecessor");
  constexpr bool COLD = MODE == kLdsTables;
  using Args = PathsArgs<PREV...>;
  auto c_b = [&]() -> const BatchInfo& {
    if constexpr (COLD) return cold_args<Args>().b;
    else return b;
  };
  auto c_qs = [&]() -> const ptd::Queues& {
    if constexpr (COLD) return cold_args<Args>().qs;
    else return qs;
  };
  const int he = iter_hash_entries(sc);
  uint32_t* tword = reinterpret_cast<uint32_t*>(lds + L.tword);
  int* lmat = reinterpret_cast<int*>(lds + L.lmat);
  uint32_t* ihash = reinterpret_cast<uint32_t*>(lds + L.ihash);
  for (int d = 1; d < b.trace_depth; ++d) iter_hash_fill(ihash + (d - 1) * he, sc, b, d);
  for (int e = threadIdx.x; MODE == 0 && e < sc.num_top; e += blockDim.x) {
    const int leaf = sc.top[e].idx, gi = sc.nodes[leaf].geom;
    tword[e] = (uint32_t)leaf | ((uint32_t)gi << 8);
    lmat[leaf & 63] = sc.geoms[gi].material;
  }
  __syncthreads();
  const int wib = threadIdx.x >> 6;
  char* wbase = lds + L.waves + wib * L.wave_bytes;
  Lanes cy = lanes_init(wbase);
  GridRings gr = grid_rings_init<false>(wbase);
  Carry<false, 1>& cb = gr.cy;
  CellRing& cr = gr.cr;
  cb.lnodes = (const __attribute__((address_space(3))) v4f*)(lnodes ? lnodes : lds), cb.lds_nodes = lnodes != nullptr;
  constexpr bool SLOTS = MODE == 0;
  char* slots = wbase + WM::slots;
  int* died = reinterpret_cast<int*>(wbase + WM::died);
  [[maybe_unused]] int* fillc = reinterpret_cast<int*>(wbase + WM::fillc);
  const int ntop = sc.num_top;
  const int wave = __builtin_amdgcn_readfirstlane(blockIdx.x * kWavesPerBlock + wib);
  const int lane = lane_id();
  died[lane] = 0;
  const uint64_t t_begin = __builtin_amdgcn_s_memrealtime();
  const DealMap dm = deal_map(qs);
  const WaveSlot even = wave_slot(wave, qs.Q, qs.W);
  int q = even.q, r = even.r, wq = even.wq;
  if (qs.deal != nullptr && qs.deal[dm.made_for()] == qs.W) {
    int at_or_before = 0;
    for (int e0 = 0; e0 < qs.Q; e0 += 64) at_or_before += (int)__popcll(ballot(e0 + lane < qs.Q && qs.deal[dm.first(e0 + lane)] <= wave));
    q = at_or_before - 1;
    const int first = qs.deal[dm.first(q)];
    r = wave - first, wq = qs.deal[dm.first(q + 1)] - first;
  }
  const Retire rt = retire_of(ret, q);
  const int64_t qbase = (int64_t)q * qs.cap;
  const int wq0 = rt.wq0, ne = b.K * wq0;
  const QueueShare qshare = queue_share(b, qs, q);
  const int my_nq = qshare.my_nq, quo = my_nq / wq0, rem = my_nq % wq0;
  auto count_of = [&](int e) { return e < ne ? (int)(uint32_t)rt.sub[e] : 0; };
  int total = 0, csum = 0;
  const bool chunk_sums = ne <= 64 * 64;
  for (int e0 = 0; e0 < ne; e0 += 256) {
    int n4[4];
#pragma unroll
    for (int j = 0; j < 4; ++j) n4[j] = count_of(e0 + 64 * j + lane);
#pragma unroll
    for (int j = 0; j < 4; ++j) {
      int sum;
      (void)wave_prefix6(n4[j], sum);
      total += sum;
      if (lane == (e0 >> 6) + j) csum = sum;
    }
  }
  if (r == 0 && lane == 0) cnt[cnt_index(qs, 1, q)] = total;
  if constexpr (SPLIT == kFirstBounce || SPLIT == kFixedSlots)
    if (r == 0 && lane == 0) cnt[cnt_index(qs, 0, q)] = b.K * qshare.my_pixels;
  const PiecePlan pieces0 = piece_plan(total, wq, b.paths_pieces, qs.deal != nullptr, chunk_sums);
  auto piece_plan_here = [&]() {
    if constexpr (COLD) return piece_plan(cold(total), wq, c_b().paths_pieces, c_qs().deal != nullptr, cold(ne) <= 64 * 64);
    else return pieces0;
  };
  [[maybe_unused]] int clist0 = 0;
  int ce = ne, cstart = total, ccnt = 0, clist = 0;
  int cord = 0;
  [[maybe_unused]] int cur_k = 0;
  [[maybe_unused]] uint32_t cur_h = 0u, next_h = 0u;
  [[maybe_unused]] int crec0 = 0;
  [[maybe_unused]] const int fbits = fixed_bits(rt.seg_cap);
  int win0 = -64;
  unsigned long long wsub = 0ull;
  auto window_to = [&](int e) {
    if (e < win0 || e >= win0 + 64) {
      win0 = e;
      wsub = (e + lane < ne) ? rt.sub[e + lane] : 0ull;
    }
  };
  auto sub_word = [&](int e) -> unsigned long long {
    const uint32_t lo32 = (uint32_t)__builtin_amdgcn_readlane((int)(uint32_t)wsub, e - win0);
    const uint32_t hi32 = (uint32_t)__builtin_amdgcn_readlane((int)(uint32_t)(wsub >> 32), e - win0);
    return ((unsigned long long)hi32 << 32) | lo32;
  };
  window_to(0);
  auto cursor_bases = [&](int first_rank) {
    const int ec = min(ce, ne - 1), ck = ec / wq0, crho = ec - ck * wq0;
    clist = ck * rt.seg_cap + sub_offset(quo, rem, crho) * 64;
    if constexpr (SPLIT != 0) clist0 = invariant_slot(clist, ck, rt.seg_cap);
    if constexpr (FIRST) cur_k = ck, cur_h = iter_hash(b.iter_first + ck, 0);
    window_to(ec);
    const int crec = clist + (int)(uint32_t)(sub_word(ec) >> 32);
    if constexpr (FIXED) crec0 = invariant_slot(crec, ck, rt.seg_cap);
    else if (lane == 0) fillc[cord & (kVisitRing - 1)] = crec + (first_rank - cstart);
  };
  auto seek = [&](int at_rank) {
    int cum = 0, e_begin = 0;
    if (COLD ? cold(ne) <= 64 * 64 : chunk_sums) {
      int all;
      const int cbefore = wave_prefix6(csum, all);
      const unsigned long long here = ballot(csum > 0 && cbefore <= at_rank && at_rank < cbefore + csum);
      if (here) {
        const int l = __builtin_ctzll(here);
        e_begin = l * 64, cum = __builtin_amdgcn_readlane(cbefore, l);
      }
    }
    for (int e0 = e_begin; e0 < ne; e0 += 64) {
      const int n = count_of(e0 + lane);
      int sum;
      const int before = wave_prefix6(n, sum);
      const unsigned long long here = ballot(n > 0 && cum + before <= at_rank && at_rank < cum + before + n);
      if (here) {
        const int l = __builtin_ctzll(here);
        ce = e0 + l, cstart = cum + __builtin_amdgcn_readlane(before, l), ccnt = __builtin_amdgcn_readlane(n, l);
        break;
      }
      cum += sum;
    }
    ++cord;
    cursor_bases(at_rank);
  };
  auto assign = [&](bool want, int rank, int& at, [[maybe_unused]] int& at0, int& rs) -> bool {
    bool pending = want;
    const int cord0 = cord;
    while (true) {
      const bool in = pending && rank < cstart + ccnt;
      if (in) at = clist + (rank - cstart), rs = cord;
      if constexpr (SPLIT != 0)
        if (in) at0 = clist0 + (rank - cstart);
      if constexpr (FIRST)
        if (in) rs = (int)(FIXED ? pack_fixed(cur_k, crec0 + (rank - cstart), fbits) : pack_visit(cur_k, cord)), next_h = cur_h;
      pending = pending && !in;
      if (!ballot(pending) || ce >= ne || (!FIXED && cord - cord0 >= kVisitsPerRefill)) break;
      cstart += ccnt;
      ccnt = 0;
      int nxt = ce + 1;
      while (nxt < ne) {
        window_to(nxt);
        const unsigned long long holds = ballot((uint32_t)wsub != 0u) & (~0ull << (nxt - win0));
        if (holds) {
          nxt = win0 + (int)__builtin_ctzll(holds);
          ccnt = (int)(uint32_t)sub_word(nxt);
          break;
        }
        nxt = win0 + 64;
      }
      ce = min(nxt, ne);
      ++cord;
      cursor_bases(cstart);
    }
    return want && !pending;
  };
  const uint32_t s_base = (uint32_t)__builtin_amdgcn_readfirstlane((int)lds_offset(slots));
  const uint32_t s16 = s_base + (uint32_t)lane * 16u, s4 = s_base + (uint32_t)kSlotTail + (uint32_t)lane * 4u;
  const ptd::Word4 *in0 = uniform_ptr(in.r + qbase), *in1 = uniform_ptr(in.r + in.stride + qbase);
  const float* in2 = uniform_ptr(reinterpret_cast<const float*>(in.r + 2 * in.stride) + 2 * qbase);
  PathRec nx;
  nx.o = nx.d = nx.c = mk(0.f, 0.f, 0.f), nx.tag = PathTag{0, 0u, 0};
  int nx_rs = 0;
  int* slot_rs = reinterpret_cast<int*>(slots + kSlotVisit) + lane;
  auto fetch = [&](int at, [[maybe_unused]] int at0, int rs) {
    if constexpr (SLOTS && SPLIT == kSplitRecords) fetch_split_to_lds(in0, in1, at, at0, s_base), *slot_rs = rs;
    else if constexpr (SLOTS) fetch_record_to_lds(in0, in1, in2, FIRST ? at0 : at, s_base), *slot_rs = rs;
    else if constexpr (SPLIT == kSplitRecords) {
      const ptd::Word4 w0 = in.r[qbase + at], w1 = in.r[in.stride + qbase + at0];
      nx.o = mk(w0.x, w0.y, w0.z), nx.d = mk(w0.w, w1.x, w1.y), nx.c = mk(w1.z, w1.w, 0.f), nx_rs = rs;
    } else nx = path_load(in, qbase + at), nx_rs = rs;
  };
  const int pix0 = b.stripe == 0 && b.pixel_begin >= 0 ? b.pixel_begin : -1;
  auto refill_pixel_map = [&]() {
    PixelMap pm{0, 0, 0, 0.f, nullptr};
    if constexpr (COLD)
      if (pix0 < 0) pm = pixel_map(c_b());
    return pm;
  };
  auto pixel_of = [&](const PixelMap& pm, int pl) {
    if constexpr (COLD) {
      if (pix0 >= 0) return pix0 + pl;
      return global_pixel(pm, pl);
    } else return global_pixel(b, pl);
  };
  [[maybe_unused]] uintptr_t top_b_scalar = (uintptr_t)sc.top_b;
  if constexpr (COLD && kFast) asm volatile("" : "+s"(top_b_scalar));
  f3 o = mk(0.f, 0.f, 0.f), d = o, c = o;
  int slot = 0, depth = 1, mark = 0, rslot = 0;
  uint32_t phash = 0u;
  bool valid = false, fresh = false, owes = false;
  bool has_next = false;
  int streamed = 0, p_hi = 0;
  [[maybe_unused]] int gj = r;
  [[maybe_unused]] uint32_t gather_time = 0u;
  [[maybe_unused]] auto gather_step = [&]() {
    if constexpr (GATHER) {
      const Args& ka = cold_args<Args>();
      const PrevGather& pg = ka.prev.p;
      const int gq = cold(q);
      const uint64_t t0 = __builtin_amdgcn_s_memrealtime();
      stream_gather_slot<kInlineGroup>(ka.b.N, pg.K, queue_share(ka.b, ka.qs, gq), ka.ret, pg.rec, pg.plane0, pg.image, gq, gj * 64 + lane);
      gj += wq;
      gather_time += (uint32_t)(__builtin_amdgcn_s_memrealtime() - t0);
    }
  };
  while (!FIRST) {
    if (streamed >= p_hi && p_hi >= 0) {
      const PiecePlan pieces = piece_plan_here();
      int nextp = -1;
      if (cord == 0) nextp = r;
      else if (pieces.needs_counter()) {
        int v = 0;
        if (lane == 0) v = atomicAdd(&c_qs().deal[deal_map(c_qs()).piece_counter(q)], 1);
        nextp = wq + __builtin_amdgcn_readfirstlane(v);
      }
      const PieceRange pr = pieces.piece_range(nextp);
      if (pr.some) {
        streamed = pr.start, p_hi = pr.end;
        seek(streamed);
      } else {
        p_hi = -1;
      }
    }
    const bool take = !valid && has_next;
    if (ballot(take || owes || (!valid && !has_next && streamed < p_hi))) {
      const PixelMap pm = refill_pixel_map();
      v4f w0, w1;
      float cz;
      int nslot, nrs;
      if constexpr (SLOTS && SPLIT == kSplitRecords) {
        asm volatile(
            "s_waitcnt vmcnt(0)\n\t"
            "ds_read_b128 %0, %3\n\t"
            "ds_read_b128 %1, %3 offset:1024\n\t"
            "ds_read_b32 %2, %4 offset:512\n\t"
            "s_waitcnt lgkmcnt(0)"
            : "=&v"(w0), "=&v"(w1), "=&v"(nrs)
            : "v"(s16), "v"(s4)
            : "memory");
        cz = 0.f, nslot = 0;
      } else if constexpr (SLOTS) {
        read_record_slot(s16, s4, w0, w1, cz, nslot, nrs);
      } else {
        w0 = v4f{nx.o.x, nx.o.y, nx.o.z, nx.d.x}, w1 = v4f{nx.d.y, nx.d.z, nx.c.x, nx.c.y}, cz = nx.c.z, nslot = nx.tag.slot, nrs = nx_rs;
      }
      if (owes) {
        rt.rec[rslot] = ptd::Word4{c.x, c.y, c.z, __int_as_float(slot & ((1 << b.slot_shift) - 1))};
        owes = false;
      }
      if constexpr (SPLIT == kSplitRecords) {
        if (take) {
          const uint32_t word = __float_as_uint(w0.w);
          const ptd::Mat* m = mats + __float_as_int(w1.w);
          nslot = kind_sample_id(word);
          o = mk(w1.x, w1.y, w1.z), d = mk(w0.x, w0.y, w0.z);
          c = mul(mk(1.0f, 1.0f, 1.0f), kind_specular(word) ? mk(m->spec[0], m->spec[1], m->spec[2]) : mk(m->color[0], m->color[1], m->color[2]));
        }
      } else if (take) o = mk(w0.x, w0.y, w0.z), d = mk(w0.w, w1.x, w1.y), c = mk(w1.z, w1.w, cz);
      if (take) {
        slot = nslot, rslot = nrs;
        phash = utilhash((uint32_t)pixel_of(pm, nslot & ((1 << b.slot_shift) - 1)));
        depth = 1;
        valid = fresh = true;
        has_next = false;
      }
      const bool lapping = ballot(valid && cord - rslot >= kVisitLap) != 0ull;
      const bool empty = !has_next && !lapping;
      const unsigned long long em = ballot(empty);
      const int rank = rank_in(em);
      const bool more = empty && streamed + rank < p_hi;
      int at = 0, at0 = 0, rs = 0;
      const bool served = assign(more, streamed + rank, at, at0, rs);
      if (served) {
        has_next = true;
        fetch(at, at0, rs);
      }
      streamed += (int)__popcll(ballot(served));
    }
    if (!ballot(valid || has_next) && p_hi < 0) break;
    bool ready;
    if constexpr (MODE == 0) {
      if (ballot(fresh)) {
        if constexpr (kFast) paths_search(cy, (cfloat4*)top_b_scalar, tword, ntop, geoms, o, d, fresh, lane, mark);
        else paths_search(cy, top, tword, ntop, geoms, o, d, fresh, lane, mark);
      }
      ready = valid && (cy.processed - mark) >= 0;
      if (cy.count > 0 && __popcll(ballot(ready)) < kPathsMinReady) {
        paths_chunk(cy, cy.count, lane, o, d, tword, geoms);
        ready = valid;
      }
    } else {
      cb.best[lane] = kNoHit;
      if constexpr (MODE == 2) grid_search<1>(cb, cr, sc, nodes, geoms, o, d, valid, lane, 0);
      else {
        PT_STAT(14, 1);
        PT_STAT(15, __popcll(ballot(valid)));
        carry_search<true, 1>(cb, top, ntop, nodes, geoms, o, d, valid, lane, 0, sc.cull_margin, sc.top_xor);
      }
      while (cb.count > 0) carry_chunk<false, 1, false, MODE == 2>(cb, min(64, cb.count), lane, nodes, geoms);
      ready = valid;
    }
    fresh = false;
    {
      ShadeIO s;
      s.o = mk(0.f, 0.f, 0.f);
      s.d = d;
      s.c = c;
      s.alive = false;
      Bounce bo;
      bo.kind = 0;
      const int k = (int)((uint32_t)slot >> b.slot_shift);
      const unsigned long long best = cy.best[lane];
      Hit h{false, -1.0f, -1, 0, mk(0.f, 0.f, 0.f), mk(0.f, 0.f, 0.f)};
      if (ready) {
        if ((uint32_t)(best >> 32) != 0x7f7fffffu) {
          h.t = __uint_as_float((uint32_t)(best >> 32));
          const float* rr = cy.rec + lane;
          h.n = mk(rr[0 * 64], rr[1 * 64], rr[2 * 64]);
          h.p = mk(rr[3 * 64], rr[4 * 64], rr[5 * 64]);
          if constexpr (MODE == 0) {
            h.mat = lmat[(uint32_t)best & 63u];
          } else {
            const ptd::Geom* G = geoms + nodes[(uint32_t)best].geom;
            h.mat = G->material;
            if (MODE == 2) h.n = finish_normal(G, h.n);
          }
        }
        const uint32_t ih = he > 0 ? ihash[(depth - 1) * he + k] : iter_hash(b.iter_first + k, depth);
        bo = shade_decide(mats, b.trace_depth, depth, ih ^ phash, h.t, h.mat, s);
      }
      const bool alive = ready && s.alive, dead = ready && !s.alive;
      if (dead) atomicAdd(&died[depth & 63], 1);
      if (dead) rslot = atomicAdd(&fillc[rslot & (kVisitRing - 1)], 1);
      if (alive) shade_bounce(bo, h.n, h.p, s);
      if (ready) {
        c = s.c;
        if (alive) o = s.o, d = s.d, depth += 1, fresh = true;
        else valid = false, owes = true;
      }
    }
  }
  if constexpr (FIRST) {
    static_assert(MODE == kLdsTables, "the first-bounce form takes its records from the refill slots of the LDS-table form");
    while (true) {
      if (ballot(fresh)) {
        if constexpr (kFast) paths_search(cy, (cfloat4*)top_b_scalar, tword, ntop, geoms, o, d, fresh, lane, mark);
        else paths_search(cy, top, tword, ntop, geoms, o, d, fresh, lane, mark);
      }
      bool ready = valid && (cy.processed - mark) >= 0;
      if (cy.count > 0 && __popcll(ballot(ready)) < kPathsMinReady) {
        paths_chunk(cy, cy.count, lane, o, d, tword, geoms);
        ready = valid;
      }
      fresh = false;
      Bounce bo;
      bo.kind = 0, bo.rng_x = 1u, bo.roughness = 0.f;
      f3 axis = mk(0.f, 0.f, 0.f);
      bool go = false;
      {
        ShadeIO s;
        s.o = mk(0.f, 0.f, 0.f);
        s.d = d;
        s.c = c;
        s.alive = false;
        const int k = (int)((uint32_t)slot >> b.slot_shift);
        const unsigned long long best = cy.best[lane];
        Hit h{false, -1.0f, -1, 0, mk(0.f, 0.f, 0.f), mk(0.f, 0.f, 0.f)};
        if (ready) {
          if ((uint32_t)(best >> 32) != 0x7f7fffffu) {
            h.t = __uint_as_float((uint32_t)(best >> 32));
            const float* rr = cy.rec + lane;
            h.n = mk(rr[0 * 64], rr[1 * 64], rr[2 * 64]);
            h.p = mk(rr[3 * 64], rr[4 * 64], rr[5 * 64]);
            h.mat = lmat[(uint32_t)best & 63u];
          }
          const uint32_t ih = he > 0 ? ihash[(depth - 1) * he + k] : iter_hash(b.iter_first + k, depth);
          bo = shade_decide(mats, b.trace_depth, depth, ih ^ phash, h.t, h.mat, s);
        }
        const bool alive = ready && s.alive, dead = ready && !s.alive;
        if (dead) atomicAdd(&died[depth & 63], 1);
        if constexpr (!FIXED)
          if (dead) rslot = atomicAdd(&fillc[rslot & (kVisitRing - 1)], 1);
        if (ready) {
          c = s.c;
          if (alive) {
            const BounceAxis a = bounce_axis(bo, h.n, h.p, d);
            o = a.o, axis = a.f, go = true;
          } else valid = false, owes = true;
        }
      }
      if (__builtin_expect(streamed >= p_hi && p_hi >= 0, 0)) {
        if constexpr (GATHER)
          if (cord != 0 && gj < my_nq) gather_step();
        const PiecePlan pieces = piece_plan_here();
        int nextp = -1;
        if (cord == 0) nextp = r;
        else if (pieces.needs_counter()) {
          int v = 0;
          if (lane == 0) v = atomicAdd(&c_qs().deal[deal_map(c_qs()).piece_counter(q)], 1);
          nextp = wq + __builtin_amdgcn_readfirstlane(v);
        }
        const PieceRange pr = pieces.piece_range(nextp);
        if (pr.some) {
          streamed = pr.start, p_hi = pr.end;
          seek(streamed);
        } else {
          p_hi = -1;
        }
      }
      const bool take = !valid && has_next;
      if (ballot(take || owes || (!valid && !has_next && streamed < p_hi))) {
        const PixelMap pm = refill_pixel_map();
        v4f w0, w1;
        float cz;
        int word, vword;
        read_record_slot(s16, s4, w0, w1, cz, word, vword);
        if (owes) {
          rt.rec[rslot] = ptd::Word4{c.x, c.y, c.z, __int_as_float(slot & ((1 << b.slot_shift) - 1))};
          owes = false;
        }
        if (take) {
          const int pl = first_pixel(word, b.slot_shift), k = FIXED ? fixed_k((uint32_t)vword, fbits) : visit_k((uint32_t)vword);
          const f3 hn = mk(w0.w, w1.x, w1.y), cam_d = mk(w1.z, w1.w, cz);
          slot = make_slot(b, k, pl), rslot = FIXED ? fixed_slot_of((uint32_t)vword, fbits, rt.seg_cap) : visit_number((uint32_t)vword);
          phash = utilhash((uint32_t)pixel_of(pm, pl));
          ShadeIO s;
          s.o = mk(0.f, 0.f, 0.f);
          s.d = cam_d;
          s.c = mk(1.0f, 1.0f, 1.0f);
          s.alive = false;
          bo = shade_decide(mats, b.trace_depth, 0, next_h ^ phash, 0.0f, first_material(word, b.slot_shift), s);
          o = mk(w0.x, w0.y, w0.z), c = s.c;
          axis = bo.kind == 1 ? bounce_reflect(cam_d, hn) : hn;
          depth = 0;
          valid = go = true;
          has_next = false;
        }
        bool lapping = false;
        if constexpr (!FIXED) lapping = ballot(valid && visit_gap(cord, rslot) >= kVisitLap) != 0ull;
        const bool empty = !has_next && !lapping;
        const unsigned long long em = ballot(empty);
        const int rank = rank_in(em);
        const bool more = empty && streamed + rank < p_hi;
        int at = 0, at0 = 0, rs = 0;
        const bool served = assign(more, streamed + rank, at, at0, rs);
        if (served) {
          has_next = true;
          fetch(at, at0, rs);
        }
        streamed += (int)__popcll(ballot(served));
      }
      if (!ballot(valid || has_next) && p_hi < 0) break;
      if (go) d = bounce_sample(bo, axis), depth += 1, fresh = true;
    }
  }
  if constexpr (GATHER) {
    while (gj < my_nq) gather_step();
    if (r == 0)
      for (int i = lane, kmax = cold_args<Args>().ret.kmax; i < kmax; i += 64) cold_args<Args>().ret.cnt[(int64_t)q * kmax + i] = 0ull;
  }
  if (lane == 0) {
    int reached = 0, rays = 0;
    int32_t* const ecnt = COLD ? cold_args<Args>().cnt : cnt;
    for (int dd = min(c_b().trace_depth - 1, 63); dd >= 2; --dd) {
      reached += died[dd];
      rays += reached;
      if (reached) atomicAdd(&ecnt[cnt_index(c_qs(), dd, q)], reached);
    }
    rays += reached + died[1];
    uint64_t spent = __builtin_amdgcn_s_memrealtime() - t_begin;
    if constexpr (GATHER) spent -= min(spent, (uint64_t)gather_time);
    const int ticks = (int)min(spent >> 6, (uint64_t)0x3ffff);
    const ptd::Queues& eq = c_qs();
    if (eq.deal != nullptr && rays) atomicAdd(&eq.deal[deal_map(eq).time(q)], ticks), atomicAdd(&eq.deal[deal_map(eq).rays(q)], rays);
  }
}

template <typename... PREV>
using PathsSignature = void (*)(decltype(PathsArgs<PREV...>::sc), decltype(PathsArgs<PREV...>::b), decltype(PathsArgs<PREV...>::qs), decltype(PathsArgs<PREV...>::cnt),
                                decltype(PathsArgs<PREV...>::in), decltype(PathsArgs<PREV...>::ret), PREV...);
static_assert(std::is_same<decltype(&k_paths<kLdsTables, kFixedSlots>), PathsSignature<>>::value, "PathsArgs does not mirror k_paths' arguments");
static_assert(std::is_same<decltype(&k_paths<kLdsTables, kFixedSlots, PrevGather>), PathsSignature<PrevGather>>::value, "PathsArgs does not mirror k_paths' arguments");
static_assert(std::is_same<decltype(PathsArgs<PrevGather>::prev.p), PrevGather>::value && std::is_standard_layout<PathsArgs<PrevGather>>::value, "PathsArgs: the gathered batch comes last");

__global__ __launch_bounds__(kBlock) void k_shade_stage(SceneTables sc, int trace_depth, int depth, int n,
                                                        const int32_t* __restrict__ iter,
                                                        const int32_t* __restrict__ pixel, ptd::HitBuf hits,
                                                        ptd::PathBuf paths, int32_t* __restrict__ alive) {
  extern __shared__ float4 lds_raw[];
  char* lds = reinterpret_cast<char*>(lds_raw);
  const ShadeLds L = shade_lds<false>(sc);
  stage16(lds + L.mats, sc.mats, mat_bytes(sc));
  __syncthreads();
  const ptd::Mat* mats = reinterpret_cast<const ptd::Mat*>(lds + L.mats);
  const int64_t HS = hits.stride;
  for (int at = blockIdx.x * blockDim.x + threadIdx.x; at < n; at += gridDim.x * blockDim.x) {
    const PathRec pr = path_load(paths, at);
    ShadeIO s;
    s.o = pr.o;
    s.d = pr.d;
    s.c = pr.c;
    s.alive = false;
    const Bounce bo = shade_decide(mats, trace_depth, depth, iter_hash(iter[at], depth) ^ utilhash((uint32_t)pixel[at]), hits.t[at], hits.mat[at], s);
    if (bo.kind) shade_bounce(bo, mk(hits.n[at], hits.n[HS + at], hits.n[2 * HS + at]),
                              mk(hits.p[at], hits.p[HS + at], hits.p[2 * HS + at]), s);
    path_store(paths, at, s.o, s.d, s.c, pr.tag);
    alive[at] = s.alive ? 1 : 0;
  }
}

#include "pt_features.inc"
#include "pt_output.inc"
#include "pt_launch.inc"
const KernelApi kApi = {
#if PT_ARITH == 0
    "exact",
#elif PT_ARITH == 1
    "fma",
#else
    "fast",
#endif
    launch_generate, launch_primary, launch_intersect, launch_shade, launch_collect, launch_count_stats,
    launch_preview, launch_save_u8, launch_shade_stage, lds_table_limit, resident_blocks_per_cu, launch_ieee_check, launch_paths,
    launch_collect_conv, launch_features, kFast ? 1 : 0, launch_intersect_grid, launch_collect_stream, launch_paths_gather,
    launch_collect_stream_planes, launch_fast_math_check};

}
}

const KernelApi* PT_API_FN() { return &PT_NS::kApi; }

#if defined(PT_WALK_STATS) && PT_ARITH == 2
}
extern "C" int pt_debug_walk_stats(unsigned long long* out) {
  unsigned long long zero[16] = {0};
  if (hipDeviceSynchronize() != hipSuccess) return -1;
  if (hipMemcpyFromSymbol(out, HIP_SYMBOL(ptk::arith_fast::g_walk_stats), sizeof(zero)) != hipSuccess) return -1;
  if (hipMemcpyToSymbol(HIP_SYMBOL(ptk::arith_fast::g_walk_stats), zero, sizeof(zero)) != hipSuccess) return -1;
  return 16;
}
namespace ptk {
#endif

}
```

cosc_4397_pathtracing_raytracing_project_amd/csrc/pt_sched.h:

```cpp
#pragma once
#include "pt_kernels.h"

#define PT_SCHED __host__ __device__ inline __attribute__((always_inline))

namespace ptk {

PT_SCHED int sched_min(int a, int b) { return a < b ? a : b; }
PT_SCHED int sched_max(int a, int b) { return a > b ? a : b; }

struct DealMap {
  int Q;
  PT_SCHED int first(int q) const { return q; }
  PT_SCHED int made_for() const { return Q; }
  PT_SCHED int time(int q) const { return Q + 1 + q; }
  PT_SCHED int strand_counter() const { return 2 * Q + 1; }
  PT_SCHED int piece_counter(int q) const { return 2 * Q + 2 + q; }
  PT_SCHED int rays(int q) const { return 3 * Q + 2 + q; }
  PT_SCHED int words() const { return 4 * Q + 2; }
};
PT_SCHED DealMap deal_map(const ptd::Queues& qs) { return DealMap{qs.Q}; }

PT_SCHED int dealt_first(int q, int W, int Q, unsigned long long work_before, unsigned long long work_total) {
  return q + (int)((unsigned long long)(W - Q) * work_before / work_total);
}
// ... 86 lines not shown
PT_SCHED bool primary_shares(int primary_share, bool aa_jitter, bool flat) { return primary_share > 1 && !aa_jitter && !flat; }
PT_SCHED bool primary_shares(const BatchInfo& b) { return primary_shares(b.primary_share, b.aa_jitter != 0, b.flat != 0); }
PT_SCHED int shared_rho(int r, int , int ) { return r; }
PT_SCHED int shared_run_cap(int primary_share) { return primary_share < 1 ? 1 : sched_min(primary_share, kShareMax); }
struct Run {
  int k0, k1;
};
PT_SCHED int shared_runs(int k0, int k1, int cap) { return (k1 - k0 + cap - 1) / cap; }
PT_SCHED Run shared_run(int k0, int k1, int cap, int i) { return Run{k0 + i * cap, sched_min(k1, k0 + (i + 1) * cap)}; }
PT_SCHED int auto_shared_pieces(int K, int , int ) {
  const int want = sched_max(2, (K + kShareMax - 1) / kShareMax);
  return sched_max(1, sched_min(want, K));
}

constexpr int kRetireEveryIteration = 1024;
struct SubSlot {
  int rho, pos;
};
PT_SCHED SubSlot sub_slot(int quo, int rem, int i) {
  const int c = i >> 6, big = rem * (quo + 1);
  const int rho = c < big ? c / (quo + 1) : rem + (c - big) / sched_max(quo, 1);
  return SubSlot{rho, i - sub_offset(quo, rem, rho) * 64};
}
PT_SCHED bool retiree_slot(const SubSlot& s, int retirees) { return s.pos < retirees; }

constexpr int kWholeRecords = 4096;
PT_SCHED int invariant_slot(int at, int k, int seg_cap) { return at - k * seg_cap; }
PT_SCHED uint32_t pack_kind(int sample_id, bool specular) { return (uint32_t)sample_id | (specular ? 0x80000000u : 0u); }
PT_SCHED int kind_sample_id(uint32_t word) { return (int)(word & 0x7fffffffu); }
PT_SCHED bool kind_specular(uint32_t word) { return (word >> 31) != 0u; }

constexpr int kNoFirstBounce = 8192;
constexpr int kSplitRecords = 1, kFirstBounce = 2;
constexpr int kSearchLdsTables = 0;
constexpr int kVisitBits = 8;
PT_SCHED uint32_t pack_visit(int k, int visit) { return ((uint32_t)k << kVisitBits) | ((uint32_t)visit & ((1u << kVisitBits) - 1u)); }
PT_SCHED int visit_k(uint32_t word) { return (int)(word >> kVisitBits); }
PT_SCHED int visit_number(uint32_t word) { return (int)(word & ((1u << kVisitBits) - 1u)); }
PT_SCHED int visit_gap(int visits_now, int visit) { return (visits_now - visit) & ((1 << kVisitBits) - 1); }
PT_SCHED bool visit_k_fits(int K) { return K <= (1 << (31 - kVisitBits)); }
PT_SCHED int pack_first(int pl, int mat, int slot_shift) { return (mat << slot_shift) | pl; }
PT_SCHED int first_pixel(int word, int slot_shift) { return word & ((1 << slot_shift) - 1); }
PT_SCHED int first_material(int word, int slot_shift) { return (int)((uint32_t)word >> slot_shift); }
PT_SCHED bool first_material_fits(int num_mats, int slot_shift) { return num_mats <= (1 << (31 - slot_shift)); }

constexpr int kPrimaryEveryBatch = 65536;

constexpr int kRecordsByVisit = 16384, kTileGather = 32768;
constexpr int kFixedSlots = 3;
PT_SCHED int fixed_slot(int k, int seg_cap, int quo, int rem, int rho, int retirees, int i) { return k * seg_cap + sub_offset(quo, rem, rho) * 64 + retirees + i; }
PT_SCHED int fixed_bits(int seg_cap) { return 32 - __builtin_clz((unsigned)(seg_cap - 1)); }
PT_SCHED uint32_t pack_fixed(int k, int in_region, int bits) { return ((uint32_t)k << bits) | (uint32_t)in_region; }
PT_SCHED int fixed_k(uint32_t word, int bits) { return (int)(word >> bits); }
PT_SCHED int fixed_slot_of(uint32_t word, int bits, int seg_cap) { return (int)(word >> bits) * seg_cap + (int)(word & ((1u << bits) - 1u)); }
PT_SCHED bool fixed_word_fits(int K, int seg_cap) { return K <= (1 << (31 - fixed_bits(seg_cap))); }
PT_SCHED int paths_split(int records, bool fixed_slots) { return records == kFirstBounce && fixed_slots ? kFixedSlots : records; }

struct FormInputs {
  int primary_share;
  bool aa_jitter, flat;
  int trace_depth, debug_flags, search_form, num_mats, slot_shift, K, seg_cap;
};
PT_SCHED FormInputs form_inputs(const BatchInfo& b, int debug_flags, int search_form, int num_mats, int seg_cap) {
  return FormInputs{b.primary_share, b.aa_jitter != 0, b.flat != 0, b.trace_depth, debug_flags, search_form, num_mats, b.slot_shift, b.K, seg_cap};
}
struct BatchForm {
  bool shares, retire_once;
  int records;
  bool fixed_slots;
  bool primary_once;
  int split;
};
PT_SCHED BatchForm batch_form(const FormInputs& in) {
  BatchForm f{};
  f.shares = primary_shares(in.primary_share, in.aa_jitter, in.flat);
  const bool invariant = f.shares && in.trace_depth >= 2;
  f.retire_once = invariant && !(in.debug_flags & kRetireEveryIteration);
  const bool splits = invariant && !(in.debug_flags & kWholeRecords);
  const bool first = splits && f.retire_once && !(in.debug_flags & kNoFirstBounce) && in.search_form == kSearchLdsTables &&
                     first_material_fits(in.num_mats, in.slot_shift) && visit_k_fits(in.K);
  f.records = first ? kFirstBounce : splits ? kSplitRecords : 0;
  f.fixed_slots = first && fixed_word_fits(in.K, in.seg_cap) && !(in.debug_flags & kRecordsByVisit);
  f.primary_once = f.fixed_slots && !(in.debug_flags & kPrimaryEveryBatch);
  f.split = paths_split(f.records, f.fixed_slots);
  return f;
}
constexpr int kRecordForms[] = {0, kSplitRecords, kFirstBounce}, kPathsSplits[] = {0, kSplitRecords, kFirstBounce, kFixedSlots};

constexpr int kGatherTile = 0, kGatherTileFixed = 1, kGatherStream = 2;
constexpr int kGatherInline = 3, kGatherEveryBatch = 131072;
constexpr int kNoSecondPlane = kGatherEveryBatch | kTileGather | kRecordsByVisit | kNoFirstBounce | kPrimaryEveryBatch;
constexpr int kFormSwitches = kTraceEveryIteration | kRetireEveryIteration | kWholeRecords | kNoSecondPlane;
struct GatherInputs {
  BatchForm form;
  bool metric, waiting;
  int waiting_plane;
  bool same_key;
  bool second_plane;
  int after, debug_flags;
  bool fused;
};
enum Closing { kCloseStream, kCloseStatsStreamPlanes, kCloseStatsConv, kCloseStatsTile, kCloseStats };
struct GatherPlan {
  int form;
  bool gathers_waiting, defers;
  int plane, reported;
  Closing closing;
};
PT_SCHED GatherPlan gather_plan(const GatherInputs& in) {
  GatherPlan p{};
  p.form = !in.form.fixed_slots ? kGatherTile : (in.debug_flags & kTileGather) || in.metric ? kGatherTileFixed : kGatherStream;
  const bool chains = p.form == kGatherStream && in.form.primary_once && in.second_plane && in.fused && !(in.debug_flags & kGatherEveryBatch);
  p.gathers_waiting = chains && in.waiting && in.same_key;
  p.defers = chains && in.after > 0;
  p.plane = p.gathers_waiting ? 1 - in.waiting_plane : p.defers ? in.after & 1 : 0;
  p.reported = p.defers ? kGatherInline : p.form;
  if (p.defers) p.closing = kCloseStats;
  else if (p.form == kGatherStream) p.closing = p.plane == 0 ? kCloseStream : kCloseStatsStreamPlanes;
  else p.closing = in.metric ? kCloseStatsConv : kCloseStatsTile;
  return p;
}

PT_SCHED int pack_paths_pieces(int count, int min_piece) { return count | min_piece << 16; }
PT_SCHED int paths_pieces_count(int word) { return word & 0xffff; }
PT_SCHED int paths_pieces_min(int word) { return word >> 16; }
struct PieceRange {
  int start, end;
  bool some;
};
struct PiecePlan {
  int total, wq, pieces_per_wave, ps_min, ps0;
  PT_SCHED bool needs_counter() const { return ps0 * wq < total; }
  PT_SCHED PieceRange piece_range(int nextp) const {
    int start = total, sz = ps0;
    if (nextp >= 0) {
      start = 0;
      int level = nextp / wq;
      const int idx = nextp - level * wq;
      for (; level > 0 && start < total; --level) start += wq * sz, sz = sched_max(sz - sz / pieces_per_wave, ps_min);
      start += idx * sz;
    }
    return start < total ? PieceRange{start, sched_min(start + sz, total), true} : PieceRange{total, total, false};
  }
};
PT_SCHED PiecePlan piece_plan(int total, int wq, int paths_pieces, bool deal_present, bool chunk_sums) {
  PiecePlan p;
  p.total = total, p.wq = wq;
  p.pieces_per_wave = deal_present && chunk_sums && paths_pieces_count(paths_pieces) > 1 ? paths_pieces_count(paths_pieces) : 1;
  p.ps_min = paths_pieces_min(paths_pieces);
  p.ps0 = sched_max((total + wq * p.pieces_per_wave - 1) / (wq * p.pieces_per_wave), p.ps_min);
  return p;
}

}
```

include/pt_amd.h:

```cpp
#ifndef PT_AMD_H
#define PT_AMD_H

#include <stdint.h>

#ifdef __cplusplus
extern "C" {
#endif

#define PT_GEOM_SPHERE 0
#define PT_GEOM_CUBE 1
#define PT_GEOM_TRIANGLE 2

typedef struct PtGeom {
  int32_t type;
  int32_t materialid;
  float transform[16];
  float inverseTransform[16];
  float invTranspose[16];
} PtGeom;

typedef struct PtMaterial {
  float color[3];
  float specular_exponent;
  float specular_color[3];
  float hasReflective;
  float hasRefractive;
  float indexOfRefraction;
  float emittance;
} PtMaterial;

typedef struct PtCamera {
  int32_t resolution[2];
  float position[3];
  float lookAt[3];
  float view[3];
  float up[3];
  float right[3];
  float fov[2];
  float pixelLength[2];
} PtCamera;

typedef struct PtBVHNode {
  float bmin[3];
  float bmax[3];
  int32_t left, right, geomIndex;
} PtBVHNode;

typedef struct PtSceneDesc {
  const PtGeom* geoms;
  int32_t num_geoms;
  const PtMaterial* materials;
  int32_t num_materials;
  PtCamera camera;
  int32_t trace_depth;
} PtSceneDesc;

typedef struct PtOptions {
  int32_t device;
  int32_t pixel_begin;
  int32_t pixel_count;
  int32_t iters_per_batch;
  int32_t num_queues;
  int32_t blocks_per_cu;
  int32_t time_kernels;
  int32_t legacy_traversal;
  int32_t debug_flags;
  int32_t unfused_primary;
  int32_t unfused_bounces;
  int32_t stripe_pixels;
  int32_t stripe_stride;
  int32_t arith;
  int32_t aa_jitter;
  int32_t convergence;
  int32_t lds_table_kb;
  int32_t primary_pieces;
  int32_t paths_pieces;
  int32_t paths_min_piece;
} PtOptions;
#define PT_PRIMARY_PIECES(pieces, share) ((int32_t)((pieces) | (share) << 16))

#define PT_ARITH_EXACT 0
#define PT_ARITH_FMA 1
#define PT_ARITH_FAST 2

#define PT_MAX_DEPTH 64
typedef struct PtStats {
  int64_t samples;
  int64_t live_rays[PT_MAX_DEPTH];
  int64_t intersect_launches;
  double intersect_ms;
  double render_ms;
  int32_t num_cus, grid_blocks, num_queues, iters_per_batch;
  int64_t device_bytes;
  int32_t primary_fused;
  int32_t bounces_fused;
  int32_t arith;
  int32_t grid_cells;
  int32_t tight_leaves;
  int32_t paths_waves;
  int32_t record_form;
  int32_t gather_form;
  int64_t primary_launches;
  int64_t inline_gathers;
} PtStats;

typedef struct PtScene PtScene;
int pt_scene_load(const char* path, int res_w, int res_h, PtScene** out);
void pt_scene_free(PtScene* s);
int pt_scene_desc(const PtScene* s, PtSceneDesc* out);
int pt_scene_iterations(const PtScene* s);
int pt_scene_orbit(PtScene* s, float dphi, float dtheta, float dzoom);
int pt_scene_camera(const PtScene* s, PtCamera* out);
int pt_scene_orbit_state(const PtScene* s, float* phi, float* theta, float* zoom);
const char* pt_scene_image_name(const PtScene* s);
int pt_scene_geom_trs(const PtScene* s, int geom, float trs[9]);
int pt_scene_set_geom_trs(PtScene* s, int geom, const float trs[9]);

int pt_build_bvh(const PtGeom* geoms, int num_geoms, PtBVHNode* out, int cap);

typedef struct PtGridInfo {
  int32_t res[3];
  float origin[3], cell_size[3], pad;
  int32_t num_cells, num_records, num_leaves;
} PtGridInfo;
typedef struct PtGridRecord {
  float bmin[3], bmax[3];
  int32_t leaf;
  int32_t neighbours;
} PtGridRecord;
int pt_build_grid(const PtGeom* geoms, int num_geoms, int forced, PtGridInfo* info, uint32_t* cell_start, PtGridRecord* records);

int pt_traversal_boxes(const PtGeom* geoms, int num_geoms, const float camera_position[3], float* boxes);

void pt_center_half_box(const float lo[3], const float hi[3], int inner, float magnitude, float center[3], float half_extent[3]);

int pt_build_transform(const float* trs, float* transform, float* inverse, float* invTranspose);

int pt_init(const PtSceneDesc* scene, const PtOptions* opt);
int pt_free(void);
int pt_render(int iter_first, int iter_count);
int pt_sync(void);
int pt_readback(float* rgb_sum_host);
int pt_readback_device(void* rgb_sum_dev);
int pt_preview_rgba8(int iterations, uint8_t* rgba_host);
int pt_preview_rgba8_device(int iterations, void* rgba_dev);
int pt_get_stats(PtStats* out);
int pt_reset_stats(void);
int pt_clear(void);
int pt_set_camera(const PtCamera* cam);
#define PT_SET_CAMERA_DEVICE_TABLES 1u
#define PT_DEVICE_TABLES_LIST 1
#define PT_DEVICE_TABLES_CELLS 2
int pt_set_camera_ex(const PtCamera* cam, uint32_t flags);
typedef struct PtSetCameraTimes {
  double tables_ms;
  double rearm_ms;
  double total_ms;
  int32_t path;
  int32_t fallback;
} PtSetCameraTimes;
int pt_get_set_camera_times(PtSetCameraTimes* out);
int pt_set_geoms(const PtGeom* geoms, int num_geoms);
typedef struct PtSetGeomsTimes {
  double build_ms;
  double upload_ms;
  double rearm_ms;
  double total_ms;
} PtSetGeomsTimes;
int pt_get_set_geoms_times(PtSetGeomsTimes* out);
typedef struct PtSetupTimes {
  double tables_ms, upload_ms, buffers_ms, probe_ms, set_camera_ms;
  int32_t set_camera_calls;
} PtSetupTimes;
int pt_get_setup_times(PtSetupTimes* out);
int pt_camera_tables_host(const PtSceneDesc* scene, const PtCamera* cam, int debug_flags, int center_half, int32_t grid_res_out[3],
                          int32_t* tight_leaves, int32_t* differing);
typedef struct PtTableNode {
  float bmin[3], bmax[3];
  int32_t skip;
  int32_t geom;
} PtTableNode;
#define PT_CAMERA_GRID_NONE 3
typedef struct PtCameraGridResult {
  int32_t res[3];
  float origin[3], cell_size[3], inv_cell_size[3], pad;
  uint32_t guard;
  int64_t num_cells;
  uint64_t refs;
  uint32_t longest;
  int32_t status;
} PtCameraGridResult;
int pt_camera_grid_host(const PtTableNode* nodes, int num_nodes, const int32_t* geom_types, int num_geoms, const float root_min[3],
                        const float root_max[3], double coord_mag, const int32_t res[3], int center_half, PtCameraGridResult* out,
                        uint32_t* start, uint64_t start_cap, PtGridRecord* items, PtGridRecord* items_b, uint64_t items_cap);
const char* pt_last_error(void);
int pt_selfcheck_ieee(int arith, int kind, uint64_t first, uint64_t count, uint32_t seed, uint64_t* mismatches);
int pt_selfcheck_fast_math(int arith, int kind, uint64_t first, uint64_t count, double* max_err);
#define PT_CONVERGENCE_WAVES 16
#define PT_CONVERGENCE_CAPACITY 65536
int pt_set_reference(const float* rgb_avg_host);
int pt_get_convergence(int iter_first, int iter_count, double* sse);
int pt_iterations_to_clean(float threshold_db, int* iteration);
float pt_psnr_from_sse(double sse, int64_t pixels);

#define PT_FEATURE_PLANES 3
int pt_render_features(int iter_first, int iter_count);
int pt_readback_features(float* planes_host);

typedef struct PtDenoiseOptions {
  int32_t levels;
  float sigma_color;
  float sigma_normal;
  float sigma_position;
  int32_t keep_albedo;
} PtDenoiseOptions;
int pt_denoise(float samples, const PtDenoiseOptions* opt, float* rgb_avg_host);
int pt_denoise_host(int w, int rows, const float* rgb_sum, const float* planes, float samples, const PtDenoiseOptions* opt, float* rgb_avg);

#define PT_NOISE_PLANES 2
#define PT_NOISE_PIXELS_PER_PARTIAL 1024
int pt_noise_fold(void);
int pt_get_noise(double* sse, int* groups, int* iterations);
int pt_readback_noise(float* planes_host);
int pt_render_until(int iter_first, int max_iters, int group_iters, float target_db, int* iters_done, float* psnr_db);
int pt_noise_fold_host(int pixels, const float* rgb_sum, float* planes, int group_iters, int groups_after, int64_t iters_after, double* sse);

#define PT_DENOISE_VARIANCE_FLOOR 1e-8f
int pt_denoise_guided(const PtDenoiseOptions* opt, float* rgb_avg_host);
int pt_denoise_guided_host(int w, int rows, const float* rgb_sum, const float* planes, const float* noise_planes, int groups, int64_t iters,
                           const PtDenoiseOptions* opt, float* rgb_avg);
int pt_denoise_guided_variance_host(int w, int rows, const float* rgb_sum, const float* planes, const float* noise_planes, int groups, int64_t iters,
                                    const PtDenoiseOptions* opt, float* var_raw, float* var_0);

int pt_adaptive_round(int iter_first, int group_iters, float fraction);
int pt_render_adaptive(int iter_first, int max_iters, int group_iters, float fraction, float target_db, int* iters_done, int64_t* samples_done,
                       float* psnr_db);
int pt_readback_adaptive(int32_t* counts);
int pt_resolve(float* rgb_avg_host);
int pt_adaptive_select_host(int w, int rows, const float* noise_planes, const int32_t* counts, int m, int32_t* list);
int pt_adaptive_merge_host(int pixels, float* rgb_sum, float* planes, int32_t* counts, const int32_t* list, int m, const float* group_sum,
                           int group_iters, double* sse);

int pt_adaptive_round_threshold(int iter_first, int group_iters, float threshold, float max_fraction, int* above, int* selected);
int pt_render_threshold(int iter_first, int max_iters, int group_iters, float threshold, float max_fraction, int min_pixels, int* iters_done,
                        int64_t* samples_done, int* above_left);
int pt_adaptive_select_threshold_host(int w, int rows, const float* noise_planes, const int32_t* counts, float threshold, int cap, int32_t* list,
                                      int* above, int* m);
int pt_adaptive_round_list(int iter_first, int group_iters, const int32_t* list_host, int m, int capacity);

int pt_denoise_adaptive(const PtDenoiseOptions* opt, float* rgb_avg_host);
int pt_denoise_adaptive_host(int w, int rows, const float* rgb_sum, const float* planes, const float* noise_planes, const int32_t* counts,
                             const PtDenoiseOptions* opt, float* rgb_avg);
int pt_denoise_adaptive_variance_host(int w, int rows, const float* rgb_sum, const float* planes, const float* noise_planes, const int32_t* counts,
                                      const PtDenoiseOptions* opt, float* var_raw, float* var_0);

#define PT_HISTORY_KEPT_PLANES 3
// ... 344 lines not shown
```

Measured before the change: 43950.

## Let idle k_paths waves migrate to other queues with pieces left

Wraps the k_paths body in a loop so that, in LDS-table mode, a wave that has drained its own queue scans every queue's piece counter and total. It picks the queue with the most remaining pieces via a DPP wave max, then joins it by bumping that queue's piece counter. This is dynamic work stealing meant to cut tail imbalance across queues within a launch. The cost is extra atomics, a cross-queue scan per wave, more register pressure from the restructured loop, and a migration counter exposed in stats, with a debug flag to disable it.

```diff
diff --git a/cosc_4397_pathtracing_raytracing_project_amd/capi.py b/cosc_4397_pathtracing_raytracing_project_amd/capi.py
--- a/cosc_4397_pathtracing_raytracing_project_amd/capi.py
+++ b/cosc_4397_pathtracing_raytracing_project_amd/capi.py
@@ -75,7 +75,8 @@
                 ("grid_blocks", C.c_int32), ("num_queues", C.c_int32), ("iters_per_batch", C.c_int32),
                 ("device_bytes", C.c_int64), ("primary_fused", C.c_int32), ("bounces_fused", C.c_int32),
                 ("arith", C.c_int32), ("grid_cells", C.c_int32), ("tight_leaves", C.c_int32), ("paths_waves", C.c_int32), ("record_form", C.c_int32),
-                ("gather_form", C.c_int32), ("primary_launches", C.c_int64), ("inline_gathers", C.c_int64)]
+                ("gather_form", C.c_int32), ("primary_launches", C.c_int64), ("inline_gathers", C.c_int64),
+                ("migrations", C.c_int64)]
 
 
 class PtDenoiseOptions(C.Structure):
diff --git a/cosc_4397_pathtracing_raytracing_project_amd/csrc/pt_api.cpp b/cosc_4397_pathtracing_raytracing_project_amd/csrc/pt_api.cpp
--- a/cosc_4397_pathtracing_raytracing_project_amd/csrc/pt_api.cpp
+++ b/cosc_4397_pathtracing_raytracing_project_amd/csrc/pt_api.cpp
@@ -15,7 +15,7 @@
 namespace {
 
 std::string g_err;
-constexpr int kDebugFlags = 16 | 32 | 64 | 256 | 512 | 2048 | ptk::kFormSwitches;
+constexpr int kDebugFlags = 16 | 32 | 64 | 256 | 512 | 2048 | ptk::kFormSwitches | ptk::kNoMigration;
 static_assert(sizeof(PtOptions) == 80, "capi.PtOptions mirrors this layout");
 static_assert(PT_CONVERGENCE_WAVES == ptk::kConvWaves, "pt_amd.h documents the size of the convergence metric's partial sums");
 }
@@ -93,6 +93,7 @@
 static ptd::Queues queues_for(const Ctx& g, int grid) {
   ptd::Queues q = g.qs;
   q.W = grid * ptk::kWavesPerBlock;
+  q.migrate = (g.debug_flags & ptk::kNoMigration) ? 0 : 1;
   return q;
 }
 
@@ -503,7 +504,7 @@
   if (ensure(g, g.d_image, image_bytes, Zero::blocking) || ensure(g, g.d_cnt, cnt_words * sizeof(int32_t), Zero::blocking) ||
       ensure(g, g.d_stats, PT_MAX_DEPTH * sizeof(*g.d_stats), Zero::blocking))
     return -1;
-  if (!(g.debug_flags & 64) && ensure(g, g.qs.deal, (size_t)ptk::deal_map(g.qs).words() * sizeof(int32_t), Zero::blocking)) return -1;
+  if (!(g.debug_flags & 64) && ensure(g, g.qs.deal, (size_t)ptk::deal_alloc_words(ptk::deal_map(g.qs)) * sizeof(int32_t), Zero::blocking)) return -1;
   if (g.conv) {
     const size_t partials = (size_t)g.K * Q * ptk::kConvWaves;
     if (ensure(g, g.d_ref, image_bytes, Zero::blocking) || ensure(g, g.d_partial, partials * sizeof(double), Zero::blocking)) return -1;
@@ -869,6 +870,11 @@
   out->inline_gathers = g.inline_gathers;
   out->primary_launches = g.primary_launches;
   out->paths_waves = 0;
+  if (g.qs.deal) {
+    int32_t moved = 0;
+    HIP_OK(hipMemcpy(&moved, g.qs.deal + ptk::deal_migrations_word(ptk::deal_map(g.qs)), sizeof(moved), hipMemcpyDeviceToHost));
+    out->migrations = moved;
+  }
   if (g.qs.deal && g.grid_paths > 0) {
     const ptk::DealMap dm = ptk::deal_map(g.qs);
     std::vector<int32_t> first((size_t)dm.made_for() + 1);
diff --git a/cosc_4397_pathtracing_raytracing_project_amd/csrc/pt_device.h b/cosc_4397_pathtracing_raytracing_project_amd/csrc/pt_device.h
--- a/cosc_4397_pathtracing_raytracing_project_amd/csrc/pt_device.h
+++ b/cosc_4397_pathtracing_raytracing_project_amd/csrc/pt_device.h
@@ -82,7 +82,7 @@
   float inv_nq;
   int32_t* deal;
   int32_t paths_W;
-  int32_t pad;
+  int32_t migrate;
 };
 
 }
diff --git a/cosc_4397_pathtracing_raytracing_project_amd/csrc/pt_kernels.hip b/cosc_4397_pathtracing_raytracing_project_amd/csrc/pt_kernels.hip
--- a/cosc_4397_pathtracing_raytracing_project_amd/csrc/pt_kernels.hip
+++ b/cosc_4397_pathtracing_raytracing_project_amd/csrc/pt_kernels.hip
@@ -1362,6 +1362,21 @@
   asm volatile("" : "+s"(v));
   return v;
 }
+PT_DEV uint32_t wave_max(uint32_t v) {
+  auto step = [](uint32_t a, int b) { return (uint32_t)b > a ? (uint32_t)b : a; };
+  uint32_t x = v;
+  x = step(x, __builtin_amdgcn_update_dpp(0, (int)x, 0x111, 0xf, 0xf, true));
+  x = step(x, __builtin_amdgcn_update_dpp(0, (int)x, 0x112, 0xf, 0xf, true));
+  x = step(x, __builtin_amdgcn_update_dpp(0, (int)x, 0x114, 0xf, 0xf, true));
+  x = step(x, __builtin_amdgcn_update_dpp(0, (int)x, 0x118, 0xf, 0xf, true));
+  x = step(x, __builtin_amdgcn_update_dpp(0, (int)x, 0x142, 0xa, 0xf, false));
+  x = step(x, __builtin_amdgcn_update_dpp(0, (int)x, 0x143, 0xc, 0xf, false));
+  return (uint32_t)__builtin_amdgcn_readlane((int)x, 63);
+}
+PT_DEV int cold_lane(int lane) {
+  asm volatile("" : "+v"(lane));
+  return lane;
+}
 template <Search MODE, int SPLIT = 0, typename... PREV>
 __global__ __launch_bounds__(kBlock, MODE == 0 ? kPathsWaves : MODE == 1 ? kPathsScanWaves : kPathsGridWaves) void k_paths(SceneTables sc, BatchInfo b, ptd::Queues qs, int32_t* __restrict__ cnt ,
                                                                ptd::PathBuf in, ptd::RetireBuf ret, PREV... prev) {
@@ -1396,6 +1411,14 @@
   auto c_qs = [&]() -> const ptd::Queues& {
     if constexpr (COLD) return cold_args<Args>().qs;
     else return qs;
+  };
+  auto c_ret = [&]() -> const ptd::RetireBuf& {
+    if constexpr (COLD) return cold_args<Args>().ret;
+    else return ret;
+  };
+  auto c_in = [&]() -> const ptd::PathBuf& {
+    if constexpr (COLD) return cold_args<Args>().in;
+    else return in;
   };
   const int he = iter_hash_entries(sc);
   uint32_t* tword = reinterpret_cast<uint32_t*>(lds + L.tword);
@@ -1423,7 +1446,7 @@
   const int wave = __builtin_amdgcn_readfirstlane(blockIdx.x * kWavesPerBlock + wib);
   const int lane = lane_id();
   died[lane] = 0;
-  const uint64_t t_begin = __builtin_amdgcn_s_memrealtime();
+  uint64_t t_begin = __builtin_amdgcn_s_memrealtime();
   const DealMap dm = deal_map(qs);
   const WaveSlot even = wave_slot(wave, qs.Q, qs.W);
   int q = even.q, r = even.r, wq = even.wq;
@@ -1434,331 +1457,284 @@
     const int first = qs.deal[dm.first(q)];
     r = wave - first, wq = qs.deal[dm.first(q + 1)] - first;
   }
-  const Retire rt = retire_of(ret, q);
-  const int64_t qbase = (int64_t)q * qs.cap;
-  const int wq0 = rt.wq0, ne = b.K * wq0;
-  const QueueShare qshare = queue_share(b, qs, q);
-  const int my_nq = qshare.my_nq, quo = my_nq / wq0, rem = my_nq % wq0;
-  auto count_of = [&](int e) { return e < ne ? (int)(uint32_t)rt.sub[e] : 0; };
-  int total = 0, csum = 0;
-  const bool chunk_sums = ne <= 64 * 64;
-  for (int e0 = 0; e0 < ne; e0 += 256) {
-    int n4[4];
-#pragma unroll
-    for (int j = 0; j < 4; ++j) n4[j] = count_of(e0 + 64 * j + lane);
-#pragma unroll
-    for (int j = 0; j < 4; ++j) {
-      int sum;
-      (void)wave_prefix6(n4[j], sum);
-      total += sum;
-      if (lane == (e0 >> 6) + j) csum = sum;
-    }
-  }
-  if (r == 0 && lane == 0) cnt[cnt_index(qs, 1, q)] = total;
-  if constexpr (SPLIT == kFirstBounce || SPLIT == kFixedSlots)
-    if (r == 0 && lane == 0) cnt[cnt_index(qs, 0, q)] = b.K * qshare.my_pixels;
-  const PiecePlan pieces0 = piece_plan(total, wq, b.paths_pieces, qs.deal != nullptr, chunk_sums);
-  auto piece_plan_here = [&]() {
-    if constexpr (COLD) return piece_plan(cold(total), wq, c_b().paths_pieces, c_qs().deal != nullptr, cold(ne) <= 64 * 64);
-    else return pieces0;
-  };
-  [[maybe_unused]] int clist0 = 0;
-  int ce = ne, cstart = total, ccnt = 0, clist = 0;
-  int cord = 0;
-  [[maybe_unused]] int cur_k = 0;
-  [[maybe_unused]] uint32_t cur_h = 0u, next_h = 0u;
-  [[maybe_unused]] int crec0 = 0;
-  [[maybe_unused]] const int fbits = fixed_bits(rt.seg_cap);
-  int win0 = -64;
-  unsigned long long wsub = 0ull;
-  auto window_to = [&](int e) {
-    if (e < win0 || e >= win0 + 64) {
-      win0 = e;
-      wsub = (e + lane < ne) ? rt.sub[e + lane] : 0ull;
-    }
-  };
-  auto sub_word = [&](int e) -> unsigned long long {
-    const uint32_t lo32 = (uint32_t)__builtin_amdgcn_readlane((int)(uint32_t)wsub, e - win0);
-    const uint32_t hi32 = (uint32_t)__builtin_amdgcn_readlane((int)(uint32_t)(wsub >> 32), e - win0);
-    return ((unsigned long long)hi32 << 32) | lo32;
-  };
-  window_to(0);
-  auto cursor_bases = [&](int first_rank) {
-    const int ec = min(ce, ne - 1), ck = ec / wq0, crho = ec - ck * wq0;
-    clist = ck * rt.seg_cap + sub_offset(quo, rem, crho) * 64;
-    if constexpr (SPLIT != 0) clist0 = invariant_slot(clist, ck, rt.seg_cap);
-    if constexpr (FIRST) cur_k = ck, cur_h = iter_hash(b.iter_first + ck, 0);
-    window_to(ec);
-    const int crec = clist + (int)(uint32_t)(sub_word(ec) >> 32);
-    if constexpr (FIXED) crec0 = invariant_slot(crec, ck, rt.seg_cap);
-    else if (lane == 0) fillc[cord & (kVisitRing - 1)] = crec + (first_rank - cstart);
-  };
-  auto seek = [&](int at_rank) {
-    int cum = 0, e_begin = 0;
-    if (COLD ? cold(ne) <= 64 * 64 : chunk_sums) {
-      int all;
-      const int cbefore = wave_prefix6(csum, all);
-      const unsigned long long here = ballot(csum > 0 && cbefore <= at_rank && at_rank < cbefore + csum);
-      if (here) {
-        const int l = __builtin_ctzll(here);
-        e_begin = l * 64, cum = __builtin_amdgcn_readlane(cbefore, l);
-      }
-    }
-    for (int e0 = e_begin; e0 < ne; e0 += 64) {
-      const int n = count_of(e0 + lane);
-      int sum;
-      const int before = wave_prefix6(n, sum);
-      const unsigned long long here = ballot(n > 0 && cum + before <= at_rank && at_rank < cum + before + n);
-      if (here) {
-        const int l = __builtin_ctzll(here);
-        ce = e0 + l, cstart = cum + __builtin_amdgcn_readlane(before, l), ccnt = __builtin_amdgcn_readlane(n, l);
-        break;
-      }
-      cum += sum;
-    }
-    ++cord;
-    cursor_bases(at_rank);
-  };
-  auto assign = [&](bool want, int rank, int& at, [[maybe_unused]] int& at0, int& rs) -> bool {
-    bool pending = want;
-    const int cord0 = cord;
-    while (true) {
-      const bool in = pending && rank < cstart + ccnt;
-      if (in) at = clist + (rank - cstart), rs = cord;
-      if constexpr (SPLIT != 0)
-        if (in) at0 = clist0 + (rank - cstart);
-      if constexpr (FIRST)
-        if (in) rs = (int)(FIXED ? pack_fixed(cur_k, crec0 + (rank - cstart), fbits) : pack_visit(cur_k, cord)), next_h = cur_h;
-      pending = pending && !in;
-      if (!ballot(pending) || ce >= ne || (!FIXED && cord - cord0 >= kVisitsPerRefill)) break;
-      cstart += ccnt;
-      ccnt = 0;
-      int nxt = ce + 1;
-      while (nxt < ne) {
-        window_to(nxt);
-        const unsigned long long holds = ballot((uint32_t)wsub != 0u) & (~0ull << (nxt - win0));
-        if (holds) {
-          nxt = win0 + (int)__builtin_ctzll(holds);
-          ccnt = (int)(uint32_t)sub_word(nxt);
-          break;
-        }
-        nxt = win0 + 64;
-      }
-      ce = min(nxt, ne);
-      ++cord;
-      cursor_bases(cstart);
-    }
-    return want && !pending;
-  };
+  constexpr bool MIGRATE = MODE == kLdsTables;
   const uint32_t s_base = (uint32_t)__builtin_amdgcn_readfirstlane((int)lds_offset(slots));
   const uint32_t s16 = s_base + (uint32_t)lane * 16u, s4 = s_base + (uint32_t)kSlotTail + (uint32_t)lane * 4u;
-  const ptd::Word4 *in0 = uniform_ptr(in.r + qbase), *in1 = uniform_ptr(in.r + in.stride + qbase);
-  const float* in2 = uniform_ptr(reinterpret_cast<const float*>(in.r + 2 * in.stride) + 2 * qbase);
-  PathRec nx;
-  nx.o = nx.d = nx.c = mk(0.f, 0.f, 0.f), nx.tag = PathTag{0, 0u, 0};
-  int nx_rs = 0;
-  int* slot_rs = reinterpret_cast<int*>(slots + kSlotVisit) + lane;
-  auto fetch = [&](int at, [[maybe_unused]] int at0, int rs) {
-    if constexpr (SLOTS && SPLIT == kSplitRecords) fetch_split_to_lds(in0, in1, at, at0, s_base), *slot_rs = rs;
-    else if constexpr (SLOTS) fetch_record_to_lds(in0, in1, in2, FIRST ? at0 : at, s_base), *slot_rs = rs;
-    else if constexpr (SPLIT == kSplitRecords) {
-      const ptd::Word4 w0 = in.r[qbase + at], w1 = in.r[in.stride + qbase + at0];
-      nx.o = mk(w0.x, w0.y, w0.z), nx.d = mk(w0.w, w1.x, w1.y), nx.c = mk(w1.z, w1.w, 0.f), nx_rs = rs;
-    } else nx = path_load(in, qbase + at), nx_rs = rs;
-  };
-  const int pix0 = b.stripe == 0 && b.pixel_begin >= 0 ? b.pixel_begin : -1;
-  auto refill_pixel_map = [&]() {
-    PixelMap pm{0, 0, 0, 0.f, nullptr};
-    if constexpr (COLD)
-      if (pix0 < 0) pm = pixel_map(c_b());
-    return pm;
-  };
-  auto pixel_of = [&](const PixelMap& pm, int pl) {
-    if constexpr (COLD) {
-      if (pix0 >= 0) return pix0 + pl;
-      return global_pixel(pm, pl);
-    } else return global_pixel(b, pl);
-  };
-  [[maybe_unused]] uintptr_t top_b_scalar = (uintptr_t)sc.top_b;
-  if constexpr (COLD && kFast) asm volatile("" : "+s"(top_b_scalar));
-  f3 o = mk(0.f, 0.f, 0.f), d = o, c = o;
-  int slot = 0, depth = 1, mark = 0, rslot = 0;
-  uint32_t phash = 0u;
-  bool valid = false, fresh = false, owes = false;
-  bool has_next = false;
-  int streamed = 0, p_hi = 0;
-  [[maybe_unused]] int gj = r;
-  [[maybe_unused]] uint32_t gather_time = 0u;
-  [[maybe_unused]] auto gather_step = [&]() {
-    if constexpr (GATHER) {
-      const Args& ka = cold_args<Args>();
-      const PrevGather& pg = ka.prev.p;
-      const int gq = cold(q);
-      const uint64_t t0 = __builtin_amdgcn_s_memrealtime();
-      stream_gather_slot<kInlineGroup>(ka.b.N, pg.K, queue_share(ka.b, ka.qs, gq), ka.ret, pg.rec, pg.plane0, pg.image, gq, gj * 64 + lane);
-      gj += wq;
-      gather_time += (uint32_t)(__builtin_amdgcn_s_memrealtime() - t0);
-    }
-  };
-  while (!FIRST) {
-    if (streamed >= p_hi && p_hi >= 0) {
-      const PiecePlan pieces = piece_plan_here();
-      int nextp = -1;
-      if (cord == 0) nextp = r;
-      else if (pieces.needs_counter()) {
-        int v = 0;
-        if (lane == 0) v = atomicAdd(&c_qs().deal[deal_map(c_qs()).piece_counter(q)], 1);
-        nextp = wq + __builtin_amdgcn_readfirstlane(v);
-      }
-      const PieceRange pr = pieces.piece_range(nextp);
-      if (pr.some) {
-        streamed = pr.start, p_hi = pr.end;
-        seek(streamed);
+  for (;;) {
+    const int slane = MIGRATE ? cold_lane(lane) : lane;
+    const Retire rt = retire_of(c_ret(), q);
+    const int64_t qbase = (int64_t)q * c_qs().cap;
+    const int wq0 = rt.wq0, ne = c_b().K * wq0;
+    const QueueShare qshare = queue_share(c_b(), c_qs(), q);
+    const int my_nq = qshare.my_nq, quo = my_nq / wq0, rem = my_nq % wq0;
+    auto count_of = [&](int e) { return e < ne ? (int)(uint32_t)rt.sub[e] : 0; };
+    int total = 0, csum = 0;
+    const bool chunk_sums = ne <= 64 * 64;
+    for (int e0 = 0; e0 < ne; e0 += 256) {
+      int n4[4];
+#pragma unroll
+      for (int j = 0; j < 4; ++j) n4[j] = count_of(e0 + 64 * j + slane);
+#pragma unroll
+      for (int j = 0; j < 4; ++j) {
+        int sum;
+        (void)wave_prefix6(n4[j], sum);
+        total += sum;
+        if (slane == (e0 >> 6) + j) csum = sum;
+      }
+    }
+    int32_t* const scnt = COLD ? cold_args<Args>().cnt : cnt;
+    if (r == 0 && slane == 0) scnt[cnt_index(c_qs(), 1, q)] = total;
+    if constexpr (SPLIT == kFirstBounce || SPLIT == kFixedSlots)
+      if (r == 0 && slane == 0) scnt[cnt_index(c_qs(), 0, q)] = c_b().K * qshare.my_pixels;
+    const PiecePlan pieces0 = piece_plan(total, wq, c_b().paths_pieces, c_qs().deal != nullptr, chunk_sums);
+    if constexpr (MIGRATE)
+      if (r >= wq && slane == 0 && pieces0.piece_range(r).some) atomicAdd(&c_qs().deal[deal_migrations_word(deal_map(c_qs()))], 1);
+    auto piece_plan_here = [&]() {
+      if constexpr (COLD) return piece_plan(cold(total), wq, c_b().paths_pieces, c_qs().deal != nullptr, cold(ne) <= 64 * 64);
+      else return pieces0;
+    };
+    [[maybe_unused]] int clist0 = 0;
+    int ce = ne, cstart = total, ccnt = 0, clist = 0;
+    int cord = 0;
+    [[maybe_unused]] int cur_k = 0;
+    [[maybe_unused]] uint32_t cur_h = 0u, next_h = 0u;
+    [[maybe_unused]] int crec0 = 0;
+    [[maybe_unused]] const int fbits = fixed_bits(rt.seg_cap);
+    int win0 = -64;
+    unsigned long long wsub = 0ull;
+    auto window_to = [&](int e) {
+      if (e < win0 || e >= win0 + 64) {
+        const int wl = MIGRATE ? cold_lane(lane) : lane;
+        win0 = e;
+        wsub = (e + wl < ne) ? rt.sub[e + wl] : 0ull;
+      }
+    };
+    auto sub_word = [&](int e) -> unsigned long long {
+      const uint32_t lo32 = (uint32_t)__builtin_amdgcn_readlane((int)(uint32_t)wsub, e - win0);
+      const uint32_t hi32 = (uint32_t)__builtin_amdgcn_readlane((int)(uint32_t)(wsub >> 32), e - win0);
+      return ((unsigned long long)hi32 << 32) | lo32;
+    };
+    window_to(0);
+    auto cursor_bases = [&](int first_rank) {
+      const int ec = min(ce, ne - 1), ck = ec / wq0, crho = ec - ck * wq0;
+      clist = ck * rt.seg_cap + sub_offset(quo, rem, crho) * 64;
+      if constexpr (SPLIT != 0) clist0 = invariant_slot(clist, ck, rt.seg_cap);
+      if constexpr (FIRST) cur_k = ck, cur_h = iter_hash(b.iter_first + ck, 0);
+      window_to(ec);
+      const int crec = clist + (int)(uint32_t)(sub_word(ec) >> 32);
+      if constexpr (FIXED) crec0 = invariant_slot(crec, ck, rt.seg_cap);
+      else if (lane == 0) fillc[cord & (kVisitRing - 1)] = crec + (first_rank - cstart);
+    };
+    auto seek = [&](int at_rank) {
+      int cum = 0, e_begin = 0;
+      if (COLD ? cold(ne) <= 64 * 64 : chunk_sums) {
+        int all;
+        const int cbefore = wave_prefix6(csum, all);
+        const unsigned long long here = ballot(csum > 0 && cbefore <= at_rank && at_rank < cbefore + csum);
+        if (here) {
+          const int l = __builtin_ctzll(here);
+          e_begin = l * 64, cum = __builtin_amdgcn_readlane(cbefore, l);
+        }
+      }
+      for (int e0 = e_begin; e0 < ne; e0 += 64) {
+        const int n = count_of(e0 + lane);
+        int sum;
+        const int before = wave_prefix6(n, sum);
+        const unsigned long long here = ballot(n > 0 && cum + before <= at_rank && at_rank < cum + before + n);
+        if (here) {
+          const int l = __builtin_ctzll(here);
+          ce = e0 + l, cstart = cum + __builtin_amdgcn_readlane(before, l), ccnt = __builtin_amdgcn_readlane(n, l);
+          break;
+        }
+        cum += sum;
+      }
+      ++cord;
+      cursor_bases(at_rank);
+    };
+    auto assign = [&](bool want, int rank, int& at, [[maybe_unused]] int& at0, int& rs) -> bool {
+      bool pending = want;
+      const int cord0 = cord;
+      while (true) {
+        const bool in = pending && rank < cstart + ccnt;
+        if (in) at = clist + (rank - cstart), rs = cord;
+        if constexpr (SPLIT != 0)
+          if (in) at0 = clist0 + (rank - cstart);
+        if constexpr (FIRST)
+          if (in) rs = (int)(FIXED ? pack_fixed(cur_k, crec0 + (rank - cstart), fbits) : pack_visit(cur_k, cord)), next_h = cur_h;
+        pending = pending && !in;
+        if (!ballot(pending) || ce >= ne || (!FIXED && cord - cord0 >= kVisitsPerRefill)) break;
+        cstart += ccnt;
+        ccnt = 0;
+        int nxt = ce + 1;
+        while (nxt < ne) {
+          window_to(nxt);
+          const unsigned long long holds = ballot((uint32_t)wsub != 0u) & (~0ull << (nxt - win0));
+          if (holds) {
+            nxt = win0 + (int)__builtin_ctzll(holds);
+            ccnt = (int)(uint32_t)sub_word(nxt);
+            break;
+          }
+          nxt = win0 + 64;
+        }
+        ce = min(nxt, ne);
+        ++cord;
+        cursor_bases(cstart);
+      }
+      return want && !pending;
+    };
+    const ptd::Word4 *in0 = uniform_ptr(c_in().r + qbase), *in1 = uniform_ptr(c_in().r + c_in().stride + qbase);
+    const float* in2 = uniform_ptr(reinterpret_cast<const float*>(c_in().r + 2 * c_in().stride) + 2 * qbase);
+    PathRec nx;
+    nx.o = nx.d = nx.c = mk(0.f, 0.f, 0.f), nx.tag = PathTag{0, 0u, 0};
+    int nx_rs = 0;
+    int* slot_rs = reinterpret_cast<int*>(slots + kSlotVisit) + lane;
+    auto fetch = [&](int at, [[maybe_unused]] int at0, int rs) {
+      if constexpr (SLOTS && SPLIT == kSplitRecords) fetch_split_to_lds(in0, in1, at, at0, s_base), *slot_rs = rs;
+      else if constexpr (SLOTS) fetch_record_to_lds(in0, in1, in2, FIRST ? at0 : at, s_base), *slot_rs = rs;
+      else if constexpr (SPLIT == kSplitRecords) {
+        const ptd::Word4 w0 = in.r[qbase + at], w1 = in.r[in.stride + qbase + at0];
+        nx.o = mk(w0.x, w0.y, w0.z), nx.d = mk(w0.w, w1.x, w1.y), nx.c = mk(w1.z, w1.w, 0.f), nx_rs = rs;
+      } else nx = path_load(in, qbase + at), nx_rs = rs;
+    };
+    const int pix0 = c_b().stripe == 0 && c_b().pixel_begin >= 0 ? c_b().pixel_begin : -1;
+    auto refill_pixel_map = [&]() {
+      PixelMap pm{0, 0, 0, 0.f, nullptr};
+      if constexpr (COLD)
+        if (pix0 < 0) pm = pixel_map(c_b());
+      return pm;
+    };
+    auto pixel_of = [&](const PixelMap& pm, int pl) {
+      if constexpr (COLD) {
+        if (pix0 >= 0) return pix0 + pl;
+        return global_pixel(pm, pl);
+      } else return global_pixel(b, pl);
+    };
+    [[maybe_unused]] uintptr_t top_b_scalar = (uintptr_t)sc.top_b;
+    if constexpr (COLD && kFast) asm volatile("" : "+s"(top_b_scalar));
+    f3 o = mk(0.f, 0.f, 0.f), d = o, c = o;
+    int slot = 0, depth = 1, mark = 0, rslot = 0;
+    uint32_t phash = 0u;
+    bool valid = false, fresh = false, owes = false;
+    bool has_next = false;
+    int streamed = 0, p_hi = 0;
+    [[maybe_unused]] int gj = r < wq ? r : 0x7fffffff;
+    [[maybe_unused]] uint32_t gather_time = 0u;
+    [[maybe_unused]] auto gather_step = [&]() {
+      if constexpr (GATHER) {
+        const Args& ka = cold_args<Args>();
+        const PrevGather& pg = ka.prev.p;
+        const int gq = cold(q);
+        const uint64_t t0 = __builtin_amdgcn_s_memrealtime();
+        stream_gather_slot<kInlineGroup>(ka.b.N, pg.K, queue_share(ka.b, ka.qs, gq), ka.ret, pg.rec, pg.plane0, pg.image, gq, gj * 64 + cold_lane(lane));
+        gj += wq;
+        gather_time += (uint32_t)(__builtin_amdgcn_s_memrealtime() - t0);
+      }
+    };
+    while (!FIRST) {
+      if (streamed >= p_hi && p_hi >= 0) {
+        const PiecePlan pieces = piece_plan_here();
+        int nextp = -1;
+        if (cord == 0) nextp = r;
+        else if (pieces.needs_counter()) {
+          int v = 0;
+          if (lane == 0) v = atomicAdd(&c_qs().deal[deal_map(c_qs()).piece_counter(q)], 1);
+          nextp = wq + __builtin_amdgcn_readfirstlane(v);
+        }
+        const PieceRange pr = pieces.piece_range(nextp);
+        if (pr.some) {
+          streamed = pr.start, p_hi = pr.end;
+          seek(streamed);
+        } else {
+          p_hi = -1;
+        }
+      }
+      const bool take = !valid && has_next;
+      if (ballot(take || owes || (!valid && !has_next && streamed < p_hi))) {
+        const PixelMap pm = refill_pixel_map();
+        v4f w0, w1;
+        float cz;
+        int nslot, nrs;
+        if constexpr (SLOTS && SPLIT == kSplitRecords) {
+          asm volatile(
+              "s_waitcnt vmcnt(0)\n\t"
+              "ds_read_b128 %0, %3\n\t"
+              "ds_read_b128 %1, %3 offset:1024\n\t"
+              "ds_read_b32 %2, %4 offset:512\n\t"
+              "s_waitcnt lgkmcnt(0)"
+              : "=&v"(w0), "=&v"(w1), "=&v"(nrs)
+              : "v"(s16), "v"(s4)
+              : "memory");
+          cz = 0.f, nslot = 0;
+        } else if constexpr (SLOTS) {
+          read_record_slot(s16, s4, w0, w1, cz, nslot, nrs);
+        } else {
+          w0 = v4f{nx.o.x, nx.o.y, nx.o.z, nx.d.x}, w1 = v4f{nx.d.y, nx.d.z, nx.c.x, nx.c.y}, cz = nx.c.z, nslot = nx.tag.slot, nrs = nx_rs;
+        }
+        if (owes) {
+          rt.rec[rslot] = ptd::Word4{c.x, c.y, c.z, __int_as_float(slot & ((1 << b.slot_shift) - 1))};
+          owes = false;
+        }
+        if constexpr (SPLIT == kSplitRecords) {
+          if (take) {
+            const uint32_t word = __float_as_uint(w0.w);
+            const ptd::Mat* m = mats + __float_as_int(w1.w);
+            nslot = kind_sample_id(word);
+            o = mk(w1.x, w1.y, w1.z), d = mk(w0.x, w0.y, w0.z);
+            c = mul(mk(1.0f, 1.0f, 1.0f), kind_specular(word) ? mk(m->spec[0], m->spec[1], m->spec[2]) : mk(m->color[0], m->color[1], m->color[2]));
+          }
+        } else if (take) o = mk(w0.x, w0.y, w0.z), d = mk(w0.w, w1.x, w1.y), c = mk(w1.z, w1.w, cz);
+        if (take) {
+          slot = nslot, rslot = nrs;
+          phash = utilhash((uint32_t)pixel_of(pm, nslot & ((1 << b.slot_shift) - 1)));
+          depth = 1;
+          valid = fresh = true;
+          has_next = false;
+        }
+        const bool lapping = ballot(valid && cord - rslot >= kVisitLap) != 0ull;
+        const bool empty = !has_next && !lapping;
+        const unsigned long long em = ballot(empty);
+        const int rank = rank_in(em);
+        const bool more = empty && streamed + rank < p_hi;
+        int at = 0, at0 = 0, rs = 0;
+        const bool served = assign(more, streamed + rank, at, at0, rs);
+        if (served) {
+          has_next = true;
+          fetch(at, at0, rs);
+        }
+        streamed += (int)__popcll(ballot(served));
+      }
+      if (!ballot(valid || has_next) && p_hi < 0) break;
+      bool ready;
+      if constexpr (MODE == 0) {
+        if (ballot(fresh)) {
+          if constexpr (kFast) paths_search(cy, (cfloat4*)top_b_scalar, tword, ntop, geoms, o, d, fresh, lane, mark);
+          else paths_search(cy, top, tword, ntop, geoms, o, d, fresh, lane, mark);
+        }
+        ready = valid && (cy.processed - mark) >= 0;
+        if (cy.count > 0 && __popcll(ballot(ready)) < kPathsMinReady) {
+          paths_chunk(cy, cy.count, lane, o, d, tword, geoms);
+          ready = valid;
+        }
       } else {
-        p_hi = -1;
-      }
-    }
-    const bool take = !valid && has_next;
-    if (ballot(take || owes || (!valid && !has_next && streamed < p_hi))) {
-      const PixelMap pm = refill_pixel_map();
-      v4f w0, w1;
-      float cz;
-      int nslot, nrs;
-      if constexpr (SLOTS && SPLIT == kSplitRecords) {
-        asm volatile(
-            "s_waitcnt vmcnt(0)\n\t"
-            "ds_read_b128 %0, %3\n\t"
-            "ds_read_b128 %1, %3 offset:1024\n\t"
-            "ds_read_b32 %2, %4 offset:512\n\t"
-            "s_waitcnt lgkmcnt(0)"
-            : "=&v"(w0), "=&v"(w1), "=&v"(nrs)
-            : "v"(s16), "v"(s4)
-            : "memory");
-        cz = 0.f, nslot = 0;
-      } else if constexpr (SLOTS) {
-        read_record_slot(s16, s4, w0, w1, cz, nslot, nrs);
-      } else {
-        w0 = v4f{nx.o.x, nx.o.y, nx.o.z, nx.d.x}, w1 = v4f{nx.d.y, nx.d.z, nx.c.x, nx.c.y}, cz = nx.c.z, nslot = nx.tag.slot, nrs = nx_rs;
-      }
-      if (owes) {
-        rt.rec[rslot] = ptd::Word4{c.x, c.y, c.z, __int_as_float(slot & ((1 << b.slot_shift) - 1))};
-        owes = false;
-      }
-      if constexpr (SPLIT == kSplitRecords) {
-        if (take) {
-          const uint32_t word = __float_as_uint(w0.w);
-          const ptd::Mat* m = mats + __float_as_int(w1.w);
-          nslot = kind_sample_id(word);
-          o = mk(w1.x, w1.y, w1.z), d = mk(w0.x, w0.y, w0.z);
-          c = mul(mk(1.0f, 1.0f, 1.0f), kind_specular(word) ? mk(m->spec[0], m->spec[1], m->spec[2]) : mk(m->color[0], m->color[1], m->color[2]));
-        }
-      } else if (take) o = mk(w0.x, w0.y, w0.z), d = mk(w0.w, w1.x, w1.y), c = mk(w1.z, w1.w, cz);
-      if (take) {
-        slot = nslot, rslot = nrs;
-        phash = utilhash((uint32_t)pixel_of(pm, nslot & ((1 << b.slot_shift) - 1)));
-        depth = 1;
-        valid = fresh = true;
-        has_next = false;
-      }
-      const bool lapping = ballot(valid && cord - rslot >= kVisitLap) != 0ull;
-      const bool empty = !has_next && !lapping;
-      const unsigned long long em = ballot(empty);
-      const int rank = rank_in(em);
-      const bool more = empty && streamed + rank < p_hi;
-      int at = 0, at0 = 0, rs = 0;
-      const bool served = assign(more, streamed + rank, at, at0, rs);
-      if (served) {
-        has_next = true;
-        fetch(at, at0, rs);
-      }
-      streamed += (int)__popcll(ballot(served));
-    }
-    if (!ballot(valid || has_next) && p_hi < 0) break;
-    bool ready;
-    if constexpr (MODE == 0) {
-      if (ballot(fresh)) {
-        if constexpr (kFast) paths_search(cy, (cfloat4*)top_b_scalar, tword, ntop, geoms, o, d, fresh, lane, mark);
-        else paths_search(cy, top, tword, ntop, geoms, o, d, fresh, lane, mark);
-      }
-      ready = valid && (cy.processed - mark) >= 0;
-      if (cy.count > 0 && __popcll(ballot(ready)) < kPathsMinReady) {
-        paths_chunk(cy, cy.count, lane, o, d, tword, geoms);
+        cb.best[lane] = kNoHit;
+        if constexpr (MODE == 2) grid_search<1>(cb, cr, sc, nodes, geoms, o, d, valid, lane, 0);
+        else {
+          PT_STAT(14, 1);
+          PT_STAT(15, __popcll(ballot(valid)));
+          carry_search<true, 1>(cb, top, ntop, nodes, geoms, o, d, valid, lane, 0, sc.cull_margin, sc.top_xor);
+        }
+        while (cb.count > 0) carry_chunk<false, 1, false, MODE == 2>(cb, min(64, cb.count), lane, nodes, geoms);
         ready = valid;
       }
-    } else {
-      cb.best[lane] = kNoHit;
-      if constexpr (MODE == 2) grid_search<1>(cb, cr, sc, nodes, geoms, o, d, valid, lane, 0);
-      else {
-        PT_STAT(14, 1);
-        PT_STAT(15, __popcll(ballot(valid)));
-        carry_search<true, 1>(cb, top, ntop, nodes, geoms, o, d, valid, lane, 0, sc.cull_margin, sc.top_xor);
-      }
-      while (cb.count > 0) carry_chunk<false, 1, false, MODE == 2>(cb, min(64, cb.count), lane, nodes, geoms);
-      ready = valid;
-    }
-    fresh = false;
-    {
-      ShadeIO s;
-      s.o = mk(0.f, 0.f, 0.f);
-      s.d = d;
-      s.c = c;
-      s.alive = false;
-      Bounce bo;
-      bo.kind = 0;
-      const int k = (int)((uint32_t)slot >> b.slot_shift);
-      const unsigned long long best = cy.best[lane];
-      Hit h{false, -1.0f, -1, 0, mk(0.f, 0.f, 0.f), mk(0.f, 0.f, 0.f)};
-      if (ready) {
-        if ((uint32_t)(best >> 32) != 0x7f7fffffu) {
-          h.t = __uint_as_float((uint32_t)(best >> 32));
-          const float* rr = cy.rec + lane;
-          h.n = mk(rr[0 * 64], rr[1 * 64], rr[2 * 64]);
-          h.p = mk(rr[3 * 64], rr[4 * 64], rr[5 * 64]);
-          if constexpr (MODE == 0) {
-            h.mat = lmat[(uint32_t)best & 63u];
-          } else {
-            const ptd::Geom* G = geoms + nodes[(uint32_t)best].geom;
-            h.mat = G->material;
-            if (MODE == 2) h.n = finish_normal(G, h.n);
-          }
-        }
-        const uint32_t ih = he > 0 ? ihash[(depth - 1) * he + k] : iter_hash(b.iter_first + k, depth);
-        bo = shade_decide(mats, b.trace_depth, depth, ih ^ phash, h.t, h.mat, s);
-      }
-      const bool alive = ready && s.alive, dead = ready && !s.alive;
-      if (dead) atomicAdd(&died[depth & 63], 1);
-      if (dead) rslot = atomicAdd(&fillc[rslot & (kVisitRing - 1)], 1);
-      if (alive) shade_bounce(bo, h.n, h.p, s);
-      if (ready) {
-        c = s.c;
-        if (alive) o = s.o, d = s.d, depth += 1, fresh = true;
-        else valid = false, owes = true;
-      }
-    }
-  }
-  if constexpr (FIRST) {
-    static_assert(MODE == kLdsTables, "the first-bounce form takes its records from the refill slots of the LDS-table form");
-    while (true) {
-      if (ballot(fresh)) {
-        if constexpr (kFast) paths_search(cy, (cfloat4*)top_b_scalar, tword, ntop, geoms, o, d, fresh, lane, mark);
-        else paths_search(cy, top, tword, ntop, geoms, o, d, fresh, lane, mark);
-      }
-      bool ready = valid && (cy.processed - mark) >= 0;
-      if (cy.count > 0 && __popcll(ballot(ready)) < kPathsMinReady) {
-        paths_chunk(cy, cy.count, lane, o, d, tword, geoms);
-        ready = valid;
-      }
       fresh = false;
-      Bounce bo;
-      bo.kind = 0, bo.rng_x = 1u, bo.roughness = 0.f;
-      f3 axis = mk(0.f, 0.f, 0.f);
-      bool go = false;
       {
         ShadeIO s;
         s.o = mk(0.f, 0.f, 0.f);
         s.d = d;
         s.c = c;
         s.alive = false;
+        Bounce bo;
+        bo.kind = 0;
         const int k = (int)((uint32_t)slot >> b.slot_shift);
         const unsigned long long best = cy.best[lane];
         Hit h{false, -1.0f, -1, 0, mk(0.f, 0.f, 0.f), mk(0.f, 0.f, 0.f)};
@@ -1768,107 +1744,197 @@
             const float* rr = cy.rec + lane;
             h.n = mk(rr[0 * 64], rr[1 * 64], rr[2 * 64]);
             h.p = mk(rr[3 * 64], rr[4 * 64], rr[5 * 64]);
-            h.mat = lmat[(uint32_t)best & 63u];
+            if constexpr (MODE == 0) {
+              h.mat = lmat[(uint32_t)best & 63u];
+            } else {
+              const ptd::Geom* G = geoms + nodes[(uint32_t)best].geom;
+              h.mat = G->material;
+              if (MODE == 2) h.n = finish_normal(G, h.n);
+            }
           }
           const uint32_t ih = he > 0 ? ihash[(depth - 1) * he + k] : iter_hash(b.iter_first + k, depth);
           bo = shade_decide(mats, b.trace_depth, depth, ih ^ phash, h.t, h.mat, s);
         }
         const bool alive = ready && s.alive, dead = ready && !s.alive;
         if (dead) atomicAdd(&died[depth & 63], 1);
-        if constexpr (!FIXED)
-          if (dead) rslot = atomicAdd(&fillc[rslot & (kVisitRing - 1)], 1);
+        if (dead) rslot = atomicAdd(&fillc[rslot & (kVisitRing - 1)], 1);
+        if (alive) shade_bounce(bo, h.n, h.p, s);
         if (ready) {
           c = s.c;
-          if (alive) {
-            const BounceAxis a = bounce_axis(bo, h.n, h.p, d);
-            o = a.o, axis = a.f, go = true;
-          } else valid = false, owes = true;
-        }
-      }
-      if (__builtin_expect(streamed >= p_hi && p_hi >= 0, 0)) {
-        if constexpr (GATHER)
-          if (cord != 0 && gj < my_nq) gather_step();
-        const PiecePlan pieces = piece_plan_here();
-        int nextp = -1;
-        if (cord == 0) nextp = r;
-        else if (pieces.needs_counter()) {
-          int v = 0;
-          if (lane == 0) v = atomicAdd(&c_qs().deal[deal_map(c_qs()).piece_counter(q)], 1);
-          nextp = wq + __builtin_amdgcn_readfirstlane(v);
-        }
-        const PieceRange pr = pieces.piece_range(nextp);
-        if (pr.some) {
-          streamed = pr.start, p_hi = pr.end;
-          seek(streamed);
-        } else {
-          p_hi = -1;
-        }
-      }
-      const bool take = !valid && has_next;
-      if (ballot(take || owes || (!valid && !has_next && streamed < p_hi))) {
-        const PixelMap pm = refill_pixel_map();
-        v4f w0, w1;
-        float cz;
-        int word, vword;
-        read_record_slot(s16, s4, w0, w1, cz, word, vword);
-        if (owes) {
-          rt.rec[rslot] = ptd::Word4{c.x, c.y, c.z, __int_as_float(slot & ((1 << b.slot_shift) - 1))};
-          owes = false;
-        }
-        if (take) {
-          const int pl = first_pixel(word, b.slot_shift), k = FIXED ? fixed_k((uint32_t)vword, fbits) : visit_k((uint32_t)vword);
-          const f3 hn = mk(w0.w, w1.x, w1.y), cam_d = mk(w1.z, w1.w, cz);
-          slot = make_slot(b, k, pl), rslot = FIXED ? fixed_slot_of((uint32_t)vword, fbits, rt.seg_cap) : visit_number((uint32_t)vword);
-          phash = utilhash((uint32_t)pixel_of(pm, pl));
+          if (alive) o = s.o, d = s.d, depth += 1, fresh = true;
+          else valid = false, owes = true;
+        }
+      }
+    }
+    if constexpr (FIRST) {
+      static_assert(MODE == kLdsTables, "the first-bounce form takes its records from the refill slots of the LDS-table form");
+      while (true) {
+        if (ballot(fresh)) {
+          if constexpr (kFast) paths_search(cy, (cfloat4*)top_b_scalar, tword, ntop, geoms, o, d, fresh, lane, mark);
+          else paths_search(cy, top, tword, ntop, geoms, o, d, fresh, lane, mark);
+        }
+        bool ready = valid && (cy.processed - mark) >= 0;
+        if (cy.count > 0 && __popcll(ballot(ready)) < kPathsMinReady) {
+          paths_chunk(cy, cy.count, lane, o, d, tword, geoms);
+          ready = valid;
+        }
+        fresh = false;
+        Bounce bo;
+        bo.kind = 0, bo.rng_x = 1u, bo.roughness = 0.f;
+        f3 axis = mk(0.f, 0.f, 0.f);
+        bool go = false;
+        {
           ShadeIO s;
           s.o = mk(0.f, 0.f, 0.f);
-          s.d = cam_d;
-          s.c = mk(1.0f, 1.0f, 1.0f);
+          s.d = d;
+          s.c = c;
           s.alive = false;
-          bo = shade_decide(mats, b.trace_depth, 0, next_h ^ phash, 0.0f, first_material(word, b.slot_shift), s);
-          o = mk(w0.x, w0.y, w0.z), c = s.c;
-          axis = bo.kind == 1 ? bounce_reflect(cam_d, hn) : hn;
-          depth = 0;
-          valid = go = true;
-          has_next = false;
-        }
-        bool lapping = false;
-        if constexpr (!FIXED) lapping = ballot(valid && visit_gap(cord, rslot) >= kVisitLap) != 0ull;
-        const bool empty = !has_next && !lapping;
-        const unsigned long long em = ballot(empty);
-        const int rank = rank_in(em);
-        const bool more = empty && streamed + rank < p_hi;
-        int at = 0, at0 = 0, rs = 0;
-        const bool served = assign(more, streamed + rank, at, at0, rs);
-        if (served) {
-          has_next = true;
-          fetch(at, at0, rs);
-        }
-        streamed += (int)__popcll(ballot(served));
-      }
-      if (!ballot(valid || has_next) && p_hi < 0) break;
-      if (go) d = bounce_sample(bo, axis), depth += 1, fresh = true;
-    }
-  }
-  if constexpr (GATHER) {
-    while (gj < my_nq) gather_step();
-    if (r == 0)
-      for (int i = lane, kmax = cold_args<Args>().ret.kmax; i < kmax; i += 64) cold_args<Args>().ret.cnt[(int64_t)q * kmax + i] = 0ull;
-  }
-  if (lane == 0) {
-    int reached = 0, rays = 0;
-    int32_t* const ecnt = COLD ? cold_args<Args>().cnt : cnt;
-    for (int dd = min(c_b().trace_depth - 1, 63); dd >= 2; --dd) {
-      reached += died[dd];
-      rays += reached;
-      if (reached) atomicAdd(&ecnt[cnt_index(c_qs(), dd, q)], reached);
-    }
-    rays += reached + died[1];
-    uint64_t spent = __builtin_amdgcn_s_memrealtime() - t_begin;
-    if constexpr (GATHER) spent -= min(spent, (uint64_t)gather_time);
-    const int ticks = (int)min(spent >> 6, (uint64_t)0x3ffff);
-    const ptd::Queues& eq = c_qs();
-    if (eq.deal != nullptr && rays) atomicAdd(&eq.deal[deal_map(eq).time(q)], ticks), atomicAdd(&eq.deal[deal_map(eq).rays(q)], rays);
+          const int k = (int)((uint32_t)slot >> b.slot_shift);
+          const unsigned long long best = cy.best[lane];
+          Hit h{false, -1.0f, -1, 0, mk(0.f, 0.f, 0.f), mk(0.f, 0.f, 0.f)};
+          if (ready) {
+            if ((uint32_t)(best >> 32) != 0x7f7fffffu) {
+              h.t = __uint_as_float((uint32_t)(best >> 32));
+              const float* rr = cy.rec + lane;
+              h.n = mk(rr[0 * 64], rr[1 * 64], rr[2 * 64]);
+              h.p = mk(rr[3 * 64], rr[4 * 64], rr[5 * 64]);
+              h.mat = lmat[(uint32_t)best & 63u];
+            }
+            const uint32_t ih = he > 0 ? ihash[(depth - 1) * he + k] : iter_hash(b.iter_first + k, depth);
+            bo = shade_decide(mats, b.trace_depth, depth, ih ^ phash, h.t, h.mat, s);
+          }
+          const bool alive = ready && s.alive, dead = ready && !s.alive;
+          if (dead) atomicAdd(&died[depth & 63], 1);
+          if constexpr (!FIXED)
+            if (dead) rslot = atomicAdd(&fillc[rslot & (kVisitRing - 1)], 1);
+          if (ready) {
+            c = s.c;
+            if (alive) {
+              const BounceAxis a = bounce_axis(bo, h.n, h.p, d);
+              o = a.o, axis = a.f, go = true;
+            } else valid = false, owes = true;
+          }
+        }
+        if (__builtin_expect(streamed >= p_hi && p_hi >= 0, 0)) {
+          if constexpr (GATHER)
+            if (cord != 0 && gj < my_nq) gather_step();
+          const PiecePlan pieces = piece_plan_here();
+          int nextp = -1;
+          if (cord == 0) nextp = r;
+          else if (pieces.needs_counter()) {
+            int v = 0;
+            if (lane == 0) v = atomicAdd(&c_qs().deal[deal_map(c_qs()).piece_counter(q)], 1);
+            nextp = wq + __builtin_amdgcn_readfirstlane(v);
+          }
+          const PieceRange pr = pieces.piece_range(nextp);
+          if (pr.some) {
+            streamed = pr.start, p_hi = pr.end;
+            seek(streamed);
+          } else {
+            p_hi = -1;
+          }
+        }
+        const bool take = !valid && has_next;
+        if (ballot(take || owes || (!valid && !has_next && streamed < p_hi))) {
+          const PixelMap pm = refill_pixel_map();
+          v4f w0, w1;
+          float cz;
+          int word, vword;
+          read_record_slot(s16, s4, w0, w1, cz, word, vword);
+          if (owes) {
+            rt.rec[rslot] = ptd::Word4{c.x, c.y, c.z, __int_as_float(slot & ((1 << b.slot_shift) - 1))};
+            owes = false;
+          }
+          if (take) {
+            const int pl = first_pixel(word, b.slot_shift), k = FIXED ? fixed_k((uint32_t)vword, fbits) : visit_k((uint32_t)vword);
+            const f3 hn = mk(w0.w, w1.x, w1.y), cam_d = mk(w1.z, w1.w, cz);
+            slot = make_slot(b, k, pl), rslot = FIXED ? fixed_slot_of((uint32_t)vword, fbits, rt.seg_cap) : visit_number((uint32_t)vword);
+            phash = utilhash((uint32_t)pixel_of(pm, pl));
+            ShadeIO s;
+            s.o = mk(0.f, 0.f, 0.f);
+            s.d = cam_d;
+            s.c = mk(1.0f, 1.0f, 1.0f);
+            s.alive = false;
+            bo = shade_decide(mats, b.trace_depth, 0, next_h ^ phash, 0.0f, first_material(word, b.slot_shift), s);
+            o = mk(w0.x, w0.y, w0.z), c = s.c;
+            axis = bo.kind == 1 ? bounce_reflect(cam_d, hn) : hn;
+            depth = 0;
+            valid = go = true;
+            has_next = false;
+          }
+          bool lapping = false;
+          if constexpr (!FIXED) lapping = ballot(valid && visit_gap(cord, rslot) >= kVisitLap) != 0ull;
+          const bool empty = !has_next && !lapping;
+          const unsigned long long em = ballot(empty);
+          const int rank = rank_in(em);
+          const bool more = empty && streamed + rank < p_hi;
+          int at = 0, at0 = 0, rs = 0;
+          const bool served = assign(more, streamed + rank, at, at0, rs);
+          if (served) {
+            has_next = true;
+            fetch(at, at0, rs);
+          }
+          streamed += (int)__popcll(ballot(served));
+        }
+        if (!ballot(valid || has_next) && p_hi < 0) break;
+        if (go) d = bounce_sample(bo, axis), depth += 1, fresh = true;
+      }
+    }
+    if constexpr (GATHER) {
+      while (gj < my_nq) gather_step();
+      if (r == 0) {
+        unsigned long long zero = 0ull;
+        asm volatile("" : "+v"(zero));
+        for (int i0 = 0, kmax = cold_args<Args>().ret.kmax; i0 < kmax; i0 += 64)
+          if (i0 + slane < kmax) cold_args<Args>().ret.cnt[(int64_t)q * kmax + i0 + slane] = zero;
+      }
+    }
+    if (lane == 0) {
+      int reached = 0, rays = 0;
+      int32_t* const ecnt = COLD ? cold_args<Args>().cnt : cnt;
+      for (int dd = min(c_b().trace_depth - 1, 63); dd >= 2; --dd) {
+        reached += died[dd];
+        rays += reached;
+        if (reached) atomicAdd(&ecnt[cnt_index(c_qs(), dd, q)], reached);
+      }
+      rays += reached + died[1];
+      uint64_t spent = __builtin_amdgcn_s_memrealtime() - t_begin;
+      if constexpr (GATHER) spent -= min(spent, (uint64_t)gather_time);
+      const uint32_t spent_lo = (uint32_t)spent, spent_hi = (uint32_t)(spent >> 32);
+      const int ticks = (spent_hi | (spent_lo >> 24)) ? 0x3ffff : (int)(spent_lo >> 6);
+      const ptd::Queues& eq = c_qs();
+      if (eq.deal != nullptr && rays) atomicAdd(&eq.deal[deal_map(eq).time(q)], ticks), atomicAdd(&eq.deal[deal_map(eq).rays(q)], rays);
+    }
+    if constexpr (!MIGRATE) break;
+    else {
+      const Args& ka = cold_args<Args>();
+      int32_t* const deal = ka.qs.deal;
+      const int Q = ka.qs.Q, W = ka.qs.W;
+      if (ka.qs.migrate == 0 || deal == nullptr || Q > kMigrateMaxQ) break;
+      const DealMap m = deal_map(ka.qs);
+      const int ln = cold_lane(lane);
+      const bool dealt = deal[m.made_for()] == W;
+      const bool sums = ka.b.K * ka.ret.wq0 <= 64 * 64;
+      uint32_t key = 0u;
+#pragma unroll 1
+      for (int e0 = 0; e0 < Q; e0 += 64) {
+        const int qq = min(e0 + ln, Q - 1);
+        const int counter = __hip_atomic_load(&deal[m.piece_counter(qq)], __ATOMIC_RELAXED, __HIP_MEMORY_SCOPE_AGENT);
+        const int tot = __hip_atomic_load(&ka.cnt[cnt_index(ka.qs, 1, qq)], __ATOMIC_RELAXED, __HIP_MEMORY_SCOPE_AGENT);
+        const int wqq = dealt ? deal[m.first(qq + 1)] - deal[m.first(qq)] : W / Q;
+        const uint32_t kq = migrate_key(pieces_left(tot, wqq, ka.b.paths_pieces, true, sums, counter), qq, q, Q);
+        key = e0 + ln < Q && kq > key ? kq : key;
+      }
+      key = wave_max(key);
+      if (key == 0u) break;
+      q = __builtin_amdgcn_readfirstlane(migrate_key_queue(key, q, Q));
+      wq = __builtin_amdgcn_readfirstlane(dealt ? deal[m.first(q + 1)] - deal[m.first(q)] : W / Q);
+      int v = 0;
+      if (ln == 0) v = atomicAdd(&deal[m.piece_counter(q)], 1);
+      r = wq + __builtin_amdgcn_readfirstlane(v);
+      died[ln] = 0;
+      t_begin = __builtin_amdgcn_s_memrealtime();
+    }
   }
 }
 
diff --git a/cosc_4397_pathtracing_raytracing_project_amd/csrc/pt_sched.h b/cosc_4397_pathtracing_raytracing_project_amd/csrc/pt_sched.h
--- a/cosc_4397_pathtracing_raytracing_project_amd/csrc/pt_sched.h
+++ b/cosc_4397_pathtracing_raytracing_project_amd/csrc/pt_sched.h
@@ -262,4 +262,37 @@
   return p;
 }
 
-}
+constexpr int kNoMigration = 262144;
+constexpr int kMigrateMaxQ = 2048;
+PT_SCHED int deal_migrations_word(const DealMap& m) { return m.words(); }
+PT_SCHED int deal_alloc_words(const DealMap& m) { return m.words() + 1; }
+PT_SCHED int pieces_in_plan(const PiecePlan& p) {
+  int n = 0, start = 0, sz = p.ps0;
+  while (start < p.total && sz > 0) {
+    const int here = sched_min(p.wq, (p.total - start + sz - 1) / sz);
+    n += here;
+    if (here < p.wq) break;
+    start += p.wq * sz;
+    const int next = sched_max(sz - sz / p.pieces_per_wave, p.ps_min);
+    if (next == sz && start < p.total) {
+      n += (p.total - start + sz - 1) / sz;
+      break;
+    }
+    sz = next;
+  }
+  return n;
+}
+PT_SCHED int pieces_left(int total, int wq, int paths_pieces, bool deal_present, bool chunk_sums, int counter) {
+  if (total <= 0 || wq <= 0 || counter < 0) return 0;
+  const PiecePlan p = piece_plan(total, wq, paths_pieces, deal_present, chunk_sums);
+  if (!p.needs_counter()) return 0;
+  return sched_max(0, pieces_in_plan(p) - wq - counter);
+}
+PT_SCHED uint32_t migrate_key(int left, int q, int home, int Q) {
+  if (left <= 0 || q == home) return 0u;
+  const int behind = (q - home - 1 + Q) % Q;
+  return ((uint32_t)sched_min(left, (1 << 20) - 1) << 11) | (uint32_t)(kMigrateMaxQ - 1 - behind);
+}
+PT_SCHED int migrate_key_queue(uint32_t key, int home, int Q) { return (home + 1 + (kMigrateMaxQ - 1 - (int)(key & (kMigrateMaxQ - 1)))) % Q; }
+
+}
diff --git a/include/pt_amd.h b/include/pt_amd.h
--- a/include/pt_amd.h
+++ b/include/pt_amd.h
@@ -102,6 +102,7 @@
   int32_t gather_form;
   int64_t primary_launches;
   int64_t inline_gathers;
+  int64_t migrations;
 } PtStats;
 
 typedef struct PtScene PtScene;
```

Measured after the change: 43120. -1.9%, worse.
